# Liz490/multimodal_alzheimer

Hardware: AMD Instinct MI355X
Metric: volumes/sec fwd+bwd, 3D-ResNet-10 @128^3 bf16, 1/2/4/8 MI355X; % HBM roofline (higher is better)
Workload: dtype bf16; 1 GPU; BASELINE config 2: Anat_CNN ResNet-10 MRI-only, 1x128^3, batch 8/GPU, weighted CE, Adam, fwd+bwd+step; global_batch=8, parallelism=dp1, step_launch=hip graph replay

## Files before the change

include/mmad.h:

```cpp
#ifndef MMAD_H
#define MMAD_H

#include <stdint.h>

#ifdef __cplusplus
extern "C" {
#endif

enum { MMAD_OK = 0, MMAD_EBADSHAPE = 1001, MMAD_EBADDTYPE = 1002, MMAD_ENULL = 1003,
       MMAD_EUNSUPPORTED = 1004, MMAD_EHIP = 2000 };

enum { MMAD_F32 = 0, MMAD_BF16 = 1, MMAD_F64 = 2, MMAD_F16 = 3, MMAD_BITS = 4 };

typedef struct mmad_conv_desc {
  int32_t n;
  int32_t ci, di, hi, wi;
  int32_t co, do_, ho, wo;
  int32_t kd, kh, kw;
  int32_t sd, sh, sw;
  int32_t pd, ph, pw;
  int32_t dd, dh, dw;
} mmad_conv_desc;

int mmad_abi_version(void);
// ... 71 lines not shown
                      float* dw, float* dbias, void* workspace, void* stream);
int mmad_conv3d_wgrad_split(const mmad_conv_desc* d, int dtype, const void* x, const void* dy,
                            float* dw, float* dbias, void* workspace, void* stream,
                            void* reduce_stream);
int mmad_stem_raw_ok(const mmad_conv_desc* d, int in_dtype, int dtype);
int mmad_conv3d_fwd_raw(const mmad_conv_desc* d, int in_dtype, const void* x, int dtype,
                        const void* w_packed, const float* bias, void* y, float* stats,
                        void* stream);
typedef struct mmad_wgrad_job {
  const float* ws;
  float* dw;
  int32_t splits, nd, k, cs, taps, tper, kind, gx, gy, gz;
} mmad_wgrad_job;
int mmad_conv3d_wgrad_deferred(const mmad_conv_desc* d, int dtype, const void* x,
                               const void* dy, float* dw, void* workspace, mmad_wgrad_job* job,
                               void* stream);
int mmad_conv3d_wgrad_raw_deferred(const mmad_conv_desc* d, int in_dtype, const void* x,
                                   int dtype, const void* dy, float* dw, void* workspace,
                                   mmad_wgrad_job* job, void* stream);
int mmad_wgrad_reduce_batch(int njobs, const mmad_wgrad_job* jobs, void* stream);
int mmad_conv3d_wgrad_raw(const mmad_conv_desc* d, int in_dtype, const void* x, int dtype,
                          const void* dy, float* dw, float* dbias, void* workspace,
                          void* stream, void* reduce_stream);
int mmad_stem_dgrad_ok(const mmad_conv_desc* d, int dtype, int out_dtype);
int64_t mmad_stem_dgrad_ws_bytes(const mmad_conv_desc* d);
int mmad_conv3d_dgrad_raw(const mmad_conv_desc* d, int dtype, const void* dy, const float* w,
                          int out_dtype, void* dx, void* ws, void* stream);

int64_t mmad_bn_stats_parts(int64_t m, int c);
int mmad_bn_stats(int dtype, int64_t m, int c, const void* y, float* parts, void* stream);
int mmad_bn_parts_fold(int c, int nparts, const float* parts, int group, float* out,
                       void* stream);
int mmad_bn_finalize(int c, int64_t count, int nparts, const float* parts,
                     const float* gamma, const float* beta, float* running_mean,
                     float* running_var, float momentum, float eps, int training,
                     float* mean, float* invstd, float* scale, float* shift,
                     int64_t* num_batches_tracked, void* stream);
typedef struct mmad_bn_fin {
  int nparts;
  const float* parts;
  const float* gamma;
  const float* beta;
  float* running_mean;
  float* running_var;
  float momentum;
  float eps;
  int training;
  float* mean;
  float* invstd;
  float* scale;
  float* shift;
  int64_t* num_batches_tracked;
} mmad_bn_fin;
int mmad_bn_finalize2(int c, int64_t count, const mmad_bn_fin* a, const mmad_bn_fin* b,
                      void* stream);
int mmad_scale_shift_act(int dtype, int64_t m, int c, const void* y, const float* scale,
                         const float* shift, const void* res, const float* rscale,
                         const float* rshift, int relu, void* out, void* stream);
int64_t mmad_bn_bwd_parts(int64_t m, int c);
int mmad_bn_bwd_reduce(int dtype, int64_t m, int c, const void* g, const void* g2,
                       const void* relu_out, const void* y, const float* mean,
                       const float* invstd, float* parts, void* stream);
int mmad_bn_bwd_finalize(int c, int64_t count, int nparts, const float* parts,
                         const float* gamma, const float* invstd, int training,
                         float* dgamma, float* dbeta, float* coef, void* stream);
int mmad_bn_bwd_apply(int dtype, int64_t m, int c, const void* g, const void* g2,
                      const void* relu_out, const void* y, const float* mean,
                      const float* invstd, const float* coef, void* dy, void* gmask_out,
                      void* stream);
int mmad_bn_bwd_reduce2(int dtype, int64_t m, int c, const void* g, const void* g2,
                        int64_t g_rows, const void* relu_out, const void* y, const float* mean,
                        const float* invstd, const void* y2,
                        const float* mean2, const float* invstd2, float* parts, float* parts2,
                        void* stream);
int mmad_bn_bwd_finalize2(int c, int64_t count, int nparts, const float* parts,
                          const float* gamma, const float* invstd, int training, float* dgamma,
                          float* dbeta, float* coef, const float* parts2, const float* gamma2,
                          const float* invstd2, int training2, float* dgamma2, float* dbeta2,
                          float* coef2, void* stream);
int mmad_bn_bwd_apply2(int dtype, int64_t m, int c, const void* g, const void* g2,
                       int64_t g_rows, const void* relu_out, const void* y, const float* mean, const float* invstd, const float* coef,
                       void* dy, const void* y2, const float* mean2, const float* invstd2,
                       const float* coef2, void* dy2, void* stream);
int mmad_bn_relu_bwd_reduce(int dtype, int64_t m, int c, const void* g, const void* y,
                            const float* mean, const float* invstd, const float* scale,
                            const float* shift, float* parts, void* stream);
int mmad_bn_relu_bwd_apply(int dtype, int64_t m, int c, const void* g, const void* y,
                           const float* mean, const float* invstd, const float* scale,
                           const float* shift, const float* coef, void* dy, void* stream);
int mmad_relu_fwd(int dtype, int64_t n, const void* x, void* y, void* stream);
int mmad_relu_bwd(int dtype, int64_t n, const void* g, const void* out, void* dx, void* stream);
int mmad_add(int dtype, int64_t n, const void* a, const void* b, void* out, void* stream);

int mmad_colsum_ws(int dtype, int64_t m, int c, const void* y, float* parts, float* out,
                   void* stream);
int mmad_maxpool3d_fwd(int dtype, int n, int c, int di, int hi, int wi, int do_, int ho,
                       int wo, int k, int s, int p, const void* x, void* y,
                       uint8_t* argmax, void* stream);
int mmad_maxpool3d_bwd(int dtype, int n, int c, int di, int hi, int wi, int do_, int ho,
                       int wo, int k, int s, int p, const void* dy, const uint8_t* argmax,
                       void* dx, void* stream);
int mmad_bnpool_fwd(int dtype, int n, int c, int di, int hi, int wi, int do_, int ho, int wo,
                    int k, int s, int p, const void* y, const float* scale, const float* shift,
                    void* out, uint8_t* argmax, void* ymax, void* stream);
int mmad_bnpool_bwd_reduce(int dtype, int64_t m, int c, const void* g, const void* g2,
                           void* gsum, const uint8_t* argmax, const void* ymax,
                           const float* mean, const float* invstd, float* parts, void* stream);
int mmad_bnpool_bwd_apply(int dtype, int n, int c, int di, int hi, int wi, int do_, int ho,
                          int wo, int k, int s, int p, const void* g, const uint8_t* argmax,
                          const void* y, const float* mean, const float* invstd,
                          const float* coef, void* dy, void* stream);
int mmad_gap_fwd(int dtype, int n, int64_t s, int c, const void* x, float* y, void* stream);
int64_t mmad_gap_fwd_ws_elems(int n, int64_t s, int c);
int mmad_gap_fwd_ws(int dtype, int n, int64_t s, int c, const void* x, float* y, float* ws,
                    void* stream);
int mmad_gap_bwd(int dtype, int n, int64_t s, int c, const float* dy, void* dx, void* stream);
int mmad_gap_bwd_compact(int dtype, int n, int64_t s, int c, const float* dy, void* dx,
                         void* stream);
int mmad_gap_parts(int n, int64_t s, int c);
int mmad_gap_partial(int dtype, int n, int64_t s, int c, const void* x, float* ws,
                     void* stream);
int mmad_gap_linear_fwd(int b, int in, int out, int parts, int64_t s, const float* ws,
                        const float* w, const float* bias, int relu, float* xs, float* y,
                        void* stream);
int mmad_linear_gap_bwd(int b, int in, int out, int64_t s, const float* x, const float* w,
                        const float* dy, const float* ymask, int rows_dtype, void* rows,
                        float* dw, float* dbias, void* stream);

int mmad_linear_fwd(int b, int in, int out, const float* x, const float* w,
                    const float* bias, int relu, float* y, void* stream);
int mmad_linear_bwd(int b, int in, int out, const float* x, const float* w,
                    const float* dy, float* dx, float* dw, float* dbias, void* stream);
int mmad_linear_bwd_ex(int b, int in, int out, const float* x, const float* w,
                       const float* dy, const float* ymask, float* dx, float* dw, float* dbias,
                       void* stream);
int mmad_concat_cols(int b, int n_in, const float* const* srcs, const int* widths,
                     float* dst, void* stream);
int mmad_split_cols(int b, int n_out, const float* src, float* const* dsts,
                    const int* widths, void* stream);

int mmad_gather_channels(int in_dtype, int nsrc, const void* const* srcs,
                         int64_t batch_stride, int64_t vox_stride, int n, int64_t vox,
                         int cpad, int out_dtype, void* dst, void* stream);
int mmad_pad_rows(int rows, int cin, int cout, const float* src, float* dst, void* stream);
int mmad_take_channel(int in_dtype, int64_t rows, int cpad, int ch, const void* src,
                      int out_dtype, void* dst, void* stream);
int mmad_concat_channels(int dtype, int64_t rows, int ca, const void* a, int cb,
                         const void* b, void* dst, void* stream);
int mmad_split_channels(int dtype, int64_t rows, int ca, int cb, const void* src, void* a,
                        void* b, void* stream);
int mmad_max2_fwd(int dtype, int64_t n, const void* a, const void* b, void* y, uint8_t* sel,
                  void* stream);
int mmad_max2_bwd(int dtype, int64_t n, const void* g, const uint8_t* sel, void* ga, void* gb,
                  void* stream);

int mmad_cast(int in_dtype, int out_dtype, int64_t n, const void* x, void* y, void* stream);
int mmad_dropout_fwd(int dtype, int64_t n, float p, uint64_t seed, const void* x, void* y,
                     uint8_t* keep, void* stream);
int mmad_dropout_fwd_dev(int dtype, int64_t n, float p, const uint64_t* seed, const void* x,
                         void* y, uint8_t* keep, void* stream);
int mmad_dropout_bwd(int dtype, int64_t n, float p, const void* g, const uint8_t* keep,
                     void* dx, void* stream);

int mmad_loss_fwd(int b, int c, const double* logits, const int64_t* labels,
                  const double* weight, double gamma, int mode, double* loss,
                  double* dlogits, void* stream);
int mmad_loss_fwd_ex(int b, int c, int logits_dtype, const void* logits,
                     const int64_t* labels, const double* weight, double gamma, int mode,
                     double* logits64, double* loss, double* dlogits, void* stream);
int mmad_loss_bwd(int64_t n, const double* dlogits, const double* gloss, const double* gout,
                  int out_dtype, void* dx, void* stream);

int mmad_bootstrap_cls_metrics(int n, int c, const double* logits, const int64_t* labels,
                               int ndraw, const int64_t* idx, float* f1, float* mcc,
                               void* stream);
int mmad_mean_std(int n, const float* v, double* out, void* stream);

int64_t mmad_norm_ws_bytes(int nscan, int64_t vox);
int mmad_mri_minmax_norm(int nscan, int64_t vox, const double* x, const double* mask,
                         double q, double* out, void* ws, double* q_out, void* stream);
int mmad_mri_zscore_norm(int nscan, int64_t vox, const double* x, const double* mask,
                         double* out, void* ws, void* stream);
int mmad_affine_norm(int64_t n, const double* x, double mean, double stdv, double* out,
                     void* stream);

#define MMAD_AUG_MAX_MOD 4
typedef struct mmad_augment_cfg {
  double flip_p[3];
  double rot_max[3];
  double scale_lo, scale_hi;
  double trans_max[3];
  double gain_lo[MMAD_AUG_MAX_MOD], gain_hi[MMAD_AUG_MAX_MOD];
  double bias_lo[MMAD_AUG_MAX_MOD], bias_hi[MMAD_AUG_MAX_MOD];
  int32_t nmod, pad_;
} mmad_augment_cfg;
int mmad_augment_draw(int b, int d, int h, int w, const mmad_augment_cfg* cfg,
                      const uint64_t* seed, double* theta, double* intensity, void* stream);
enum { MMAD_PAD_ZEROS = 0, MMAD_PAD_BORDER = 1 };
int mmad_affine_resample3d(int b, int d, int h, int w, const double* x, const double* theta,
                           const double* gain_bias, int64_t gb_stride, int padding,
                           double* out, void* stream);

int64_t mmad_cache_stride_bytes(int kind, int64_t vox);
int64_t mmad_cache_ws_bytes(void);
// ... 16 lines not shown
```

multimodal_alzheimer_amd/_lib.py:

```python
import ctypes as C
import os

import torch

_PKG = os.path.dirname(os.path.abspath(__file__))
LIB_PATH = os.environ.get("MMAD_LIB_PATH") or os.path.join(_PKG, "libmmad_hip.so")

F32, BF16, F64 = 0, 1, 2
F16, BITS = 3, 4
EUNSUPPORTED = 1004
EHIP = 2000
_HIP_OOM = 2

_vp, _i32, _i64, _f32, _f64, _u64 = C.c_void_p, C.c_int, C.c_int64, C.c_float, C.c_double, C.c_uint64


class ConvDesc(C.Structure):
    _fields_ = [(n, C.c_int32) for n in (
        "n", "ci", "di", "hi", "wi", "co", "do_", "ho", "wo", "kd", "kh", "kw",
        "sd", "sh", "sw", "pd", "ph", "pw", "dd", "dh", "dw")]


class PackJob(C.Structure):
    _fields_ = ([("w", C.c_void_p), ("w_packed", C.c_void_p)] +
# ... 19 lines not shown
class BnFin(C.Structure):
    _fields_ = ([("nparts", C.c_int32)] +
                [(n, C.c_void_p) for n in ("parts", "gamma", "beta", "running_mean",
                                           "running_var")] +
                [("momentum", C.c_float), ("eps", C.c_float), ("training", C.c_int32)] +
                [(n, C.c_void_p) for n in ("mean", "invstd", "scale", "shift",
                                           "num_batches_tracked")])


class WgradJob(C.Structure):
    _fields_ = ([("ws", C.c_void_p), ("dw", C.c_void_p)] +
                [(n, C.c_int32) for n in ("splits", "nd", "k", "cs", "taps", "tper", "kind",
                                          "gx", "gy", "gz")])


AUG_MAX_MOD = 4
PAD_ZEROS, PAD_BORDER = 0, 1


class AugmentCfg(C.Structure):
    _fields_ = ([("flip_p", C.c_double * 3), ("rot_max", C.c_double * 3),
                 ("scale_lo", C.c_double), ("scale_hi", C.c_double),
                 ("trans_max", C.c_double * 3)] +
                [(n, C.c_double * AUG_MAX_MOD) for n in ("gain_lo", "gain_hi", "bias_lo",
                                                         "bias_hi")] +
                [("nmod", C.c_int32), ("pad_", C.c_int32)])


_P = C.POINTER(ConvDesc)
_PJ = C.POINTER(PackJob)
_PD = C.POINTER(PackDual)
_PA = C.POINTER(AdamJob)
_SIGS = {
    "mmad_abi_version": (_i32, []),
    "mmad_strerror": (C.c_char_p, [_i32]),
    "mmad_set_kernel_variant": (_i32, [C.c_char_p, _i32]),
    "mmad_conv_packed_elems": (_i64, [_P, _i32, _i32]),
    "mmad_conv_pack_weight": (_i32, [_P, _i32, _vp, _vp, _i32, _vp]),
    "mmad_conv_pack_job": (_i32, [_P, _i32, _i32, _vp, _vp, _i64, _PJ]),
    "mmad_pack_job_tiles": (_i64, [_PJ]),
    "mmad_conv_pack_batch": (_i32, [_i32, _i32, _vp, _i64, _vp]),
    "mmad_conv_pack_dual_job": (_i32, [_P, _i32, _vp, _vp, _vp, _i64, _PD]),
    "mmad_pack_dual_tiles": (_i64, [_PD]),
    "mmad_conv_pack_dual_batch": (_i32, [_i32, _i32, _vp, _i64, _vp]),
    "mmad_adam_job_tiles": (_i64, [_PA]),
    "mmad_adam_repack": (_i32, [_i32, _vp, _vp, _i64, _vp, _vp]),
    "mmad_conv_unfolded_elems": (_i64, [_P]),
    "mmad_conv_unfold_input": (_i32, [_P, _i32, _vp, _i32, _vp, _vp]),
    "mmad_conv3d_stats_rows": (_i64, [_P, _i32]),
    "mmad_conv3d_fwd": (_i32, [_P, _i32, _vp, _vp, _vp, _vp, _vp, _vp]),
    "mmad_conv3d_dgrad": (_i32, [_P, _i32, _vp, _vp, _vp, _vp]),
    "mmad_conv3d_dgrad_bnsum_rows": (_i64, [_P, _i32]),
    "mmad_conv3d_dgrad_bnsum": (_i32, [_P, _i32] + [_vp] * 10),
    "mmad_conv3d_wgrad_workspace": (_i64, [_P, _i32]),
    "mmad_conv3d_wgrad": (_i32, [_P, _i32, _vp, _vp, _vp, _vp, _vp, _vp]),
    "mmad_conv3d_wgrad_split": (_i32, [_P, _i32, _vp, _vp, _vp, _vp, _vp, _vp, _vp]),
    "mmad_conv3d_wgrad_deferred": (_i32, [_P, _i32, _vp, _vp, _vp, _vp,
                                          C.POINTER(WgradJob), _vp]),
    "mmad_conv3d_wgrad_raw_deferred": (_i32, [_P, _i32, _vp, _i32, _vp, _vp, _vp,
                                              C.POINTER(WgradJob), _vp]),
    "mmad_wgrad_reduce_batch": (_i32, [_i32, C.POINTER(WgradJob), _vp]),
    "mmad_stem_raw_ok": (_i32, [_P, _i32, _i32]),
    "mmad_conv3d_fwd_raw": (_i32, [_P, _i32, _vp, _i32, _vp, _vp, _vp, _vp, _vp]),
    "mmad_conv3d_wgrad_raw": (_i32, [_P, _i32, _vp, _i32, _vp, _vp, _vp, _vp, _vp, _vp]),
    "mmad_stem_dgrad_ok": (_i32, [_P, _i32, _i32]),
    "mmad_stem_dgrad_ws_bytes": (_i64, [_P]),
    "mmad_conv3d_dgrad_raw": (_i32, [_P, _i32, _vp, _vp, _i32, _vp, _vp, _vp]),
    "mmad_bn_stats_parts": (_i64, [_i64, _i32]),
    "mmad_bn_stats": (_i32, [_i32, _i64, _i32, _vp, _vp, _vp]),
    "mmad_bn_parts_fold": (_i32, [_i32, _i32, _vp, _i32, _vp, _vp]),
    "mmad_bn_finalize": (_i32, [_i32, _i64, _i32, _vp, _vp, _vp, _vp, _vp, _f32, _f32, _i32,
                                _vp, _vp, _vp, _vp, _vp, _vp]),
    "mmad_bn_finalize2": (_i32, [_i32, _i64, C.POINTER(BnFin), C.POINTER(BnFin), _vp]),
    "mmad_scale_shift_act": (_i32, [_i32, _i64, _i32, _vp, _vp, _vp, _vp, _vp, _vp, _i32, _vp,
                                    _vp]),
    "mmad_bn_bwd_parts": (_i64, [_i64, _i32]),
    "mmad_bn_bwd_reduce": (_i32, [_i32, _i64, _i32] + [_vp] * 8),
    "mmad_bn_bwd_finalize": (_i32, [_i32, _i64, _i32, _vp, _vp, _vp, _i32, _vp, _vp, _vp, _vp]),
    "mmad_bn_bwd_apply": (_i32, [_i32, _i64, _i32] + [_vp] * 10),
    "mmad_bn_bwd_reduce2": (_i32, [_i32, _i64, _i32, _vp, _vp, _i64] + [_vp] * 10),
    "mmad_bn_bwd_finalize2": (_i32, [_i32, _i64, _i32, _vp, _vp, _vp, _i32, _vp, _vp, _vp,
                                     _vp, _vp, _vp, _i32, _vp, _vp, _vp, _vp]),
    "mmad_bn_bwd_apply2": (_i32, [_i32, _i64, _i32, _vp, _vp, _i64] + [_vp] * 12),
    "mmad_relu_fwd": (_i32, [_i32, _i64, _vp, _vp, _vp]),
    "mmad_relu_bwd": (_i32, [_i32, _i64, _vp, _vp, _vp, _vp]),
    "mmad_colsum_ws": (_i32, [_i32, _i64, _i32, _vp, _vp, _vp, _vp]),
    "mmad_add": (_i32, [_i32, _i64, _vp, _vp, _vp, _vp]),
    "mmad_maxpool3d_fwd": (_i32, [_i32] * 12 + [_vp, _vp, _vp, _vp]),
    "mmad_maxpool3d_bwd": (_i32, [_i32] * 12 + [_vp, _vp, _vp, _vp]),
    "mmad_bnpool_fwd": (_i32, [_i32] * 12 + [_vp] * 7),
    "mmad_bnpool_bwd_reduce": (_i32, [_i32, _i64, _i32] + [_vp] * 9),
    "mmad_bnpool_bwd_apply": (_i32, [_i32] * 12 + [_vp] * 8),
    "mmad_gap_fwd": (_i32, [_i32, _i32, _i64, _i32, _vp, _vp, _vp]),
    "mmad_gap_fwd_ws_elems": (_i64, [_i32, _i64, _i32]),
    "mmad_conv3d_fwd_ex": (_i32, [_P, _i32, _vp, _vp, _vp, _vp, _i32, _vp, _vp, _vp]),
    "mmad_conv_pack_weight_scaled": (_i32, [_P, _i32, _vp, _vp, _vp, _i32, _vp]),
    "mmad_bn_fold": (_i32, [_i32, _vp, _vp, _vp, _vp, _f32, _vp, _vp, _vp, _vp]),
    "mmad_norm_ws_bytes": (_i64, [_i32, _i64]),
    "mmad_mri_minmax_norm": (_i32, [_i32, _i64, _vp, _vp, _f64, _vp, _vp, _vp, _vp]),
    "mmad_mri_zscore_norm": (_i32, [_i32, _i64, _vp, _vp, _vp, _vp, _vp]),
    "mmad_affine_norm": (_i32, [_i64, _vp, _f64, _f64, _vp, _vp]),
    "mmad_gap_fwd_ws": (_i32, [_i32, _i32, _i64, _i32, _vp, _vp, _vp, _vp]),
    "mmad_gap_bwd": (_i32, [_i32, _i32, _i64, _i32, _vp, _vp, _vp]),
    "mmad_gap_bwd_compact": (_i32, [_i32, _i32, _i64, _i32, _vp, _vp, _vp]),
    "mmad_gap_parts": (_i32, [_i32, _i64, _i32]),
    "mmad_gap_partial": (_i32, [_i32, _i32, _i64, _i32, _vp, _vp, _vp]),
    "mmad_gap_linear_fwd": (_i32, [_i32, _i32, _i32, _i32, _i64, _vp, _vp, _vp, _i32, _vp,
                                   _vp, _vp]),
    "mmad_linear_gap_bwd": (_i32, [_i32, _i32, _i32, _i64, _vp, _vp, _vp, _vp, _i32, _vp, _vp,
                                   _vp, _vp]),
    "mmad_linear_fwd": (_i32, [_i32, _i32, _i32, _vp, _vp, _vp, _i32, _vp, _vp]),
    "mmad_linear_bwd": (_i32, [_i32, _i32, _i32, _vp, _vp, _vp, _vp, _vp, _vp, _vp]),
    "mmad_linear_bwd_ex": (_i32, [_i32, _i32, _i32] + [_vp] * 8),
    "mmad_concat_cols": (_i32, [_i32, _i32, _vp, _vp, _vp, _vp]),
    "mmad_split_cols": (_i32, [_i32, _i32, _vp, _vp, _vp, _vp]),
    "mmad_cast": (_i32, [_i32, _i32, _i64, _vp, _vp, _vp]),
    "mmad_dropout_fwd": (_i32, [_i32, _i64, _f32, _u64, _vp, _vp, _vp, _vp]),
    "mmad_dropout_fwd_dev": (_i32, [_i32, _i64, _f32, _vp, _vp, _vp, _vp, _vp]),
    "mmad_dropout_bwd": (_i32, [_i32, _i64, _f32, _vp, _vp, _vp, _vp]),
    "mmad_loss_fwd": (_i32, [_i32, _i32, _vp, _vp, _vp, _f64, _i32, _vp, _vp, _vp]),
    "mmad_loss_fwd_ex": (_i32, [_i32, _i32, _i32, _vp, _vp, _vp, _f64, _i32, _vp, _vp, _vp,
                                _vp]),
    "mmad_loss_bwd": (_i32, [_i64, _vp, _vp, _vp, _i32, _vp, _vp]),
    "mmad_gather_channels": (_i32, [_i32, _i32, _vp, _i64, _i64, _i32, _i64, _i32, _i32, _vp,
                                    _vp]),
    "mmad_pad_rows": (_i32, [_i32, _i32, _i32, _vp, _vp, _vp]),
    "mmad_take_channel": (_i32, [_i32, _i64, _i32, _i32, _vp, _i32, _vp, _vp]),
    "mmad_concat_channels": (_i32, [_i32, _i64, _i32, _vp, _i32, _vp, _vp, _vp]),
    "mmad_split_channels": (_i32, [_i32, _i64, _i32, _i32, _vp, _vp, _vp, _vp]),
    "mmad_max2_fwd": (_i32, [_i32, _i64, _vp, _vp, _vp, _vp, _vp]),
    "mmad_max2_bwd": (_i32, [_i32, _i64, _vp, _vp, _vp, _vp, _vp]),
    "mmad_bootstrap_cls_metrics": (_i32, [_i32, _i32, _vp, _vp, _i32, _vp, _vp, _vp, _vp]),
    "mmad_mean_std": (_i32, [_i32, _vp, _vp, _vp]),
    "mmad_bn_relu_bwd_reduce": (_i32, [_i32, _i64, _i32] + [_vp] * 8),
    "mmad_bn_relu_bwd_apply": (_i32, [_i32, _i64, _i32] + [_vp] * 9),
    "mmad_augment_draw": (_i32, [_i32, _i32, _i32, _i32, C.POINTER(AugmentCfg), _vp, _vp, _vp,
                                 _vp]),
    "mmad_affine_resample3d": (_i32, [_i32, _i32, _i32, _i32, _vp, _vp, _vp, _i64, _i32, _vp,
                                      _vp]),
    "mmad_cache_stride_bytes": (_i64, [_i32, _i64]),
    "mmad_cache_ws_bytes": (_i64, []),
    "mmad_cache_store": (_i32, [_i32, _i32, _i64, _vp, _vp, _i64, _i64, _vp, _vp, _vp]),
    "mmad_cache_pack_mask": (_i32, [_i32, _i64, _vp, _vp, _i64, _i64, _vp, _vp, _vp]),
    "mmad_cache_fetch": (_i32, [_i32, _i32, _i64] + [_i32] * 6 + [_vp, _vp, _vp, _i64, _vp, _vp,
                                                                 _vp]),
    "mmad_cache_fetch_rows": (_i32, [_i32, _i64, _i32, _vp, _vp, _vp, _vp, _i64, _vp, _vp, _vp,
                                     _vp]),
}
EXPORTS = tuple(_SIGS)

_lib = None


class MMADError(RuntimeError):
    pass


def load():
    global _lib
    if _lib is None:
        if not os.path.exists(LIB_PATH):
            raise MMADError(f"{LIB_PATH} is missing: build it with "
                            "`python -m multimodal_alzheimer_amd._build` (hipcc, gfx950)")
        lib = C.CDLL(LIB_PATH)
        for name, (res, args) in _SIGS.items():
            fn = getattr(lib, name)
            fn.restype, fn.argtypes = res, args
        if lib.mmad_abi_version() != 1:
            raise MMADError("libmmad_hip.so ABI version mismatch")
        _lib = lib
    return _lib


def check(rc, what=""):
    if rc == 0:
        return
    msg = load().mmad_strerror(rc).decode()
    if rc == EHIP + _HIP_OOM:
        raise torch.OutOfMemoryError(f"{what}: {msg}")
    raise MMADError(f"{what} failed ({rc}): {msg}")


def call(name, *args):
    check(getattr(load(), name)(*args), name)


_cur_dev = torch._C._cuda_getDevice
_raw_stream = torch._C._cuda_getCurrentRawStream

# ... 29 lines not shown
```

multimodal_alzheimer_amd/csrc/bn.hip:

```cpp
#include "common.h"

constexpr int COLSUM_ROWS = 4;

namespace {

struct PartPlan {
  int64_t rpp;
  int nparts;
};
PartPlan part_plan(int64_t M) {
  int n = (int)std::min<int64_t>(1024, std::max<int64_t>(1, cdiv(M, 64)));
  const int64_t rpp = cdiv(M, n);
  return {rpp, (int)cdiv(M, rpp)};
}

#ifndef BN_FOLD_PROBE
#define BN_FOLD_PROBE 0
#endif
#if BN_FOLD_PROBE
__device__ int g_fold_cnt[4096];
__device__ float g_fold_sink[4096];
#endif

template <typename T, int MODE, int V, bool DUAL = false, bool G2 = false, bool GB = false>
__global__ __launch_bounds__(256) void colsum_kernel(int64_t M, int C, int64_t rpp,
                                                     const T* __restrict__ y,
                                                     const T* __restrict__ g,
                                                     const T* __restrict__ relu_out,
                                                     const float* __restrict__ mean,
                                                     const float* __restrict__ invstd,
                                                     float* __restrict__ parts,
                                                     const uint8_t* __restrict__ act,
                                                     const float* __restrict__ msc,
                                                     const float* __restrict__ msh,
                                                     const T* __restrict__ y2 = nullptr,
                                                     const float* __restrict__ mean2 = nullptr,
                                                     const float* __restrict__ invstd2 = nullptr,
                                                     float* __restrict__ parts2 = nullptr,
                                                     const T* __restrict__ g2 = nullptr,
                                                     T* __restrict__ gsum = nullptr,
                                                     uint32_t gS = 0) {
  static_assert(!DUAL || MODE == 1, "dual partial sums: BN backward with a relu_out mask");
  static_assert(!GB || (DUAL && V == Chunk<T>::N), "broadcast g: the pair kernel, 16-byte rows");
  __shared__ float red[DUAL ? 3 : 2][2048];
  const int tid = threadIdx.x;
  const int CC = C / (int)gridDim.y;
  const int cb = (int)blockIdx.y * CC;
  const int lpr = CC / V;
  const int rpar = 256 / lpr;
  const int cl = tid % lpr, rl = tid / lpr;
  const int64_t r0 = (int64_t)blockIdx.x * rpp;
  const int64_t r1 = min(M, r0 + rpp);
  float s[V], q[V], q2[V];
#pragma unroll
  for (int e = 0; e < V; ++e) { s[e] = 0.f; q[e] = 0.f; q2[e] = 0.f; }
  if (rl < rpar) {
    float mu[V], is[V], sc[V], sh[V], mu2[V], is2[V];
    if (MODE == 1 || MODE == 3 || MODE == 4) {
#pragma unroll
      for (int e = 0; e < V; ++e) { mu[e] = mean[cb + cl * V + e]; is[e] = invstd[cb + cl * V + e]; }
    }
    if constexpr (DUAL) {
#pragma unroll
      for (int e = 0; e < V; ++e) {
        mu2[e] = mean2[cb + cl * V + e];
        is2[e] = invstd2[cb + cl * V + e];
      }
    }
    if (MODE == 4) {
#pragma unroll
      for (int e = 0; e < V; ++e) { sc[e] = msc[cb + cl * V + e]; sh[e] = msh[cb + cl * V + e]; }
    }
    auto accum = [&](int64_t i, float* yv, float* gv, const float* ov, const float* y2v) {
      if (MODE == 1 || MODE == 3 || MODE == 4) {
        if (MODE == 4) {
#pragma unroll
          for (int e = 0; e < V; ++e) gv[e] = bn_affine(yv[e], sc[e], sh[e]) > 0.f ? gv[e] : 0.f;
        } else if (MODE == 3) {
#pragma unroll
          for (int e = 0; e < V; ++e) gv[e] = (act[i + e] & 0x80) ? gv[e] : 0.f;
        } else if (relu_out != nullptr) {
#pragma unroll
          for (int e = 0; e < V; ++e) gv[e] = ov[e] > 0.f ? gv[e] : 0.f;
        }
#pragma unroll
        for (int e = 0; e < V; ++e) {
          s[e] += gv[e];
          q[e] += gv[e] * ((yv[e] - mu[e]) * is[e]);
        }
        if constexpr (DUAL) {
#pragma unroll
          for (int e = 0; e < V; ++e) q2[e] += gv[e] * ((y2v[e] - mu2[e]) * is2[e]);
        }
      } else {
#pragma unroll
        for (int e = 0; e < V; ++e) {
          s[e] += yv[e];
          if (MODE == 0) q[e] += yv[e] * yv[e];
        }
      }
    };
    constexpr bool NEED_G = MODE == 1 || MODE == 3 || MODE == 4;
    int64_t r = r0 + rl;
    if constexpr (V == Chunk<T>::N) {
      constexpr int U = COLSUM_ROWS;
      for (; r + (U - 1) * rpar < r1; r += U * rpar) {
        u32x4 yr[U], gr[U], orr[U], y2r[U], g2r[U];
#pragma unroll
        for (int u = 0; u < U; ++u) {
          const int64_t i = (r + u * rpar) * C + cb + cl * V;
          yr[u] = *reinterpret_cast<const u32x4*>(y + i);
          if constexpr (GB)
            gr[u] = *reinterpret_cast<const u32x4*>(
                g + (int64_t)((uint32_t)(r + u * rpar) / gS) * C + cb + cl * V);
          else if (NEED_G)
            gr[u] = *reinterpret_cast<const u32x4*>(g + i);
          if (NEED_G && G2) g2r[u] = *reinterpret_cast<const u32x4*>(g2 + i);
          if (MODE == 1 && relu_out != nullptr)
            orr[u] = *reinterpret_cast<const u32x4*>(relu_out + i);
          if constexpr (DUAL) y2r[u] = *reinterpret_cast<const u32x4*>(y2 + i);
        }
#pragma unroll
        for (int u = 0; u < U; ++u) {
          const int64_t i = (r + u * rpar) * C + cb + cl * V;
          float yv[V], gv[V], ov[V], y2v[V];
          Chunk<T>::load(reinterpret_cast<const T*>(&yr[u]), yv);
          if (NEED_G) Chunk<T>::load(reinterpret_cast<const T*>(&gr[u]), gv);
          if constexpr (NEED_G && G2) {
            float hv[V];
            Chunk<T>::load(reinterpret_cast<const T*>(&g2r[u]), hv);
#pragma unroll
            for (int e = 0; e < V; ++e) gv[e] = as_stored<T>(gv[e] + hv[e]);
            if constexpr (MODE == 3) Chunk<T>::store(gsum + i, gv);
          }
          if (MODE == 1 && relu_out != nullptr)
            Chunk<T>::load(reinterpret_cast<const T*>(&orr[u]), ov);
          if constexpr (DUAL) Chunk<T>::load(reinterpret_cast<const T*>(&y2r[u]), y2v);
          accum(i, yv, gv, ov, y2v);
        }
      }
    }
    for (; r < r1; r += rpar) {
      const int64_t i = r * C + cb + cl * V;
      float yv[V], gv[V], ov[V], y2v[V];
      if constexpr (V == Chunk<T>::N) Chunk<T>::load(y + i, yv);
      else for (int e = 0; e < V; ++e) yv[e] = Elt<T>::ld(y, i + e);
      if (NEED_G) {
        if constexpr (GB) Chunk<T>::load(g + (int64_t)((uint32_t)r / gS) * C + cb + cl * V, gv);
        else if constexpr (V == Chunk<T>::N) Chunk<T>::load(g + i, gv);
        else for (int e = 0; e < V; ++e) gv[e] = Elt<T>::ld(g, i + e);
        if constexpr (G2) {
          float hv[V];
          if constexpr (V == Chunk<T>::N) Chunk<T>::load(g2 + i, hv);
          else for (int e = 0; e < V; ++e) hv[e] = Elt<T>::ld(g2, i + e);
#pragma unroll
          for (int e = 0; e < V; ++e) gv[e] = as_stored<T>(gv[e] + hv[e]);
          if constexpr (MODE == 3) {
            if constexpr (V == Chunk<T>::N) Chunk<T>::store(gsum + i, gv);
            else for (int e = 0; e < V; ++e) Elt<T>::st(gsum, i + e, gv[e]);
          }
        }
        if (MODE == 1 && relu_out != nullptr) {
          if constexpr (V == Chunk<T>::N) Chunk<T>::load(relu_out + i, ov);
          else for (int e = 0; e < V; ++e) ov[e] = Elt<T>::ld(relu_out, i + e);
        }
      }
      if constexpr (DUAL) {
        if constexpr (V == Chunk<T>::N) Chunk<T>::load(y2 + i, y2v);
        else for (int e = 0; e < V; ++e) y2v[e] = Elt<T>::ld(y2, i + e);
      }
      accum(i, yv, gv, ov, y2v);
    }
#pragma unroll
    for (int e = 0; e < V; ++e) {
      red[0][rl * CC + cl * V + e] = s[e];
      red[1][rl * CC + cl * V + e] = q[e];
      if constexpr (DUAL) red[DUAL ? 2 : 0][rl * CC + cl * V + e] = q2[e];
    }
  }
  __syncthreads();
  for (int c = tid; c < CC; c += 256) {
    float ss = 0.f, qq = 0.f, q2q = 0.f;
    for (int k = 0; k < rpar; ++k) {
      ss += red[0][k * CC + c];
      qq += red[1][k * CC + c];
      if constexpr (DUAL) q2q += red[DUAL ? 2 : 0][k * CC + c];
    }
    parts[((int64_t)blockIdx.x * 2) * C + cb + c] = ss;
    parts[((int64_t)blockIdx.x * 2 + 1) * C + cb + c] = qq;
    if constexpr (DUAL) {
      parts2[((int64_t)blockIdx.x * 2) * C + cb + c] = ss;
      parts2[((int64_t)blockIdx.x * 2 + 1) * C + cb + c] = q2q;
    }
  }
#if BN_FOLD_PROBE
  __shared__ int last;
  const int ngx = ((int)gridDim.x + 31) >> 5;
  const int grp = (int)blockIdx.y * ngx + ((int)blockIdx.x >> 5);
  const int gsize = min(32, (int)gridDim.x - (((int)blockIdx.x >> 5) << 5));
  __threadfence();
  __syncthreads();
  if (tid == 0) last = atomicAdd(&g_fold_cnt[grp & 4095], 1) == gsize - 1;
  __syncthreads();
  if (last) {
    __threadfence();
    for (int c = tid; c < CC; c += 256) {
      float ss = 0.f, qq = 0.f;
      const int p0 = ((int)blockIdx.x >> 5) << 5;
      for (int k = 0; k < gsize; ++k) {
        ss += parts[((int64_t)(p0 + k) * 2) * C + cb + c];
        qq += parts[((int64_t)(p0 + k) * 2 + 1) * C + cb + c];
      }
      g_fold_sink[(grp * 64 + c) & 4095] = ss + qq;
    }
    if (tid == 0) g_fold_cnt[grp & 4095] = 0;
  }
#endif
}

__global__ void parts_fold_kernel(int C, int nparts, int group, const float* __restrict__ in,
                                  float* __restrict__ out) {
  const int o = blockIdx.x;
  for (int c = threadIdx.x; c < 2 * C; c += blockDim.x) {
    float s = 0.f;
    const int p1 = min(nparts, (o + 1) * group);
#pragma unroll 8
    for (int p = o * group; p < p1; ++p) s += in[(int64_t)p * 2 * C + c];
    out[(int64_t)o * 2 * C + c] = s;
  }
}

template <typename T, int MODE>
int launch_colsum(int64_t M, int C, const void* y, const void* g, const void* ro,
                  const float* mean, const float* invstd, float* parts, hipStream_t st,
                  const uint8_t* act = nullptr, const float* msc = nullptr,
                  const float* msh = nullptr, const void* g2 = nullptr,
                  void* gsum = nullptr) {
  const PartPlan pp = part_plan(M);
  constexpr int VEC = Chunk<T>::N;
  dim3 grid((unsigned)pp.nparts);
  int slabs = 1;
  while (C % (slabs * 2 * VEC) == 0 && C / (slabs * VEC) > 256) slabs *= 2;
#define COLSUM(VV, G)                                                                       \
  hipLaunchKernelGGL((colsum_kernel<T, MODE, VV, false, G>), grid, dim3(256), 0, st, M, C, \
                     pp.rpp, (const T*)y, (const T*)g, (const T*)ro, mean, invstd, parts, act, \
// ... 137 lines not shown
  if (conv_bias) sh += conv_bias[c] * sc;
  scale[c] = sc;
  bias[c] = sh;
}

__device__ __forceinline__ void bwd_finalize(int C, int64_t count, int nparts,
                                             const float* parts, const float* gamma,
                                             const float* invstd, int training, float* dgamma,
                                             float* dbeta, float* coef, double* sm) {
  const int c = blockIdx.x * FC + (threadIdx.x % FC);
  const bool own = threadIdx.x < FC && c < C;
  float gm = 1.f, is = 0.f;
  if (own) {
    if (gamma) gm = gamma[c];
    is = invstd[c];
  }
  double S, Q;
  sum_parts(c, C, nparts, parts, sm, S, Q);
  if (!own) return;
  if (dbeta) dbeta[c] = (float)S;
  if (dgamma) dgamma[c] = (float)Q;
  const double k0 = (double)gm * is;
  coef[c] = (float)k0;
  coef[C + c] = training ? (float)(k0 * S / (double)count) : 0.f;
  coef[2 * C + c] = training ? (float)(k0 * Q / (double)count) : 0.f;
}

__global__ __launch_bounds__(1024) void bn_bwd_finalize_kernel(
    int C, int64_t count, int nparts, const float* __restrict__ parts,
    const float* __restrict__ gamma, const float* __restrict__ invstd, int training,
    float* dgamma, float* dbeta, float* coef) {
  __shared__ double sm[2048];
  bwd_finalize(C, count, nparts, parts, gamma, invstd, training, dgamma, dbeta, coef, sm);
}

struct BwdFin {
  const float* parts;
  const float* gamma;
  const float* invstd;
  int training;
  float* dgamma;
  float* dbeta;
  float* coef;
};

__global__ __launch_bounds__(1024) void bn_bwd_finalize2_kernel(int C, int64_t count,
                                                                int nparts, BwdFin a, BwdFin b) {
  __shared__ double sm[2048];
  const BwdFin& f = blockIdx.y ? b : a;
  bwd_finalize(C, count, nparts, f.parts, f.gamma, f.invstd, f.training, f.dgamma, f.dbeta,
               f.coef, sm);
}

__global__ void sum_only_finalize_kernel(int C, int nparts, const float* __restrict__ parts,
                                         float* out) {
  __shared__ double sm[2048];
  const int c = blockIdx.x * FC + (threadIdx.x % FC);
  double S, Q;
  sum_parts(c, C, nparts, parts, sm, S, Q);
  if (threadIdx.x >= FC || c >= C) return;
  out[c] = (float)S;
}

template <typename T, int RES>
__global__ void scale_shift_act_kernel(int64_t M, int C, const T* __restrict__ y,
                                       const float* __restrict__ scale,
                                       const float* __restrict__ shift,
                                       const T* __restrict__ res,
                                       const float* __restrict__ rscale,
                                       const float* __restrict__ rshift, int relu,
                                       T* __restrict__ out) {
  constexpr int N = Chunk<T>::N;
  const int64_t nchunks = M * C / N;
  for (int64_t q = blockIdx.x * (int64_t)blockDim.x + threadIdx.x; q < nchunks;
       q += (int64_t)gridDim.x * blockDim.x) {
    const int64_t i0 = q * N;
    const int c0 = (int)(i0 % C);
    float v[N], r[N];
    Chunk<T>::load(y + i0, v);
    if (RES) Chunk<T>::load(res + i0, r);
#pragma unroll
    for (int e = 0; e < N; ++e) {
      const int c = c0 + e;
      float o = bn_affine(v[e], scale[c], shift[c]);
      if (RES == 1) o += r[e];
      if (RES == 2) o += r[e] * rscale[c] + rshift[c];
      v[e] = relu ? fmaxf(o, 0.f) : o;
    }
    Chunk<T>::store(out + i0, v);
  }
}

template <int N>
__device__ __forceinline__ void ld_params(const float* __restrict__ p, float* v) {
#pragma unroll
  for (int h = 0; h < N / 4; ++h) {
    const f32x4 c = *reinterpret_cast<const f32x4*>(p + 4 * h);
    v[4 * h] = c[0]; v[4 * h + 1] = c[1]; v[4 * h + 2] = c[2]; v[4 * h + 3] = c[3];
  }
}

template <typename T, int RES>
__global__ __launch_bounds__(256) void scale_shift_act_fc_kernel(
    int64_t nchunks, int cpr, const T* __restrict__ y, const float* __restrict__ scale,
    const float* __restrict__ shift, const T* __restrict__ res, const float* __restrict__ rscale,
    const float* __restrict__ rshift, int relu, T* __restrict__ out) {
  constexpr int N = Chunk<T>::N;
  const int64_t t0 = (int64_t)blockIdx.x * 256 + threadIdx.x;
  const int64_t stride = (int64_t)gridDim.x * 256;
  const int c0 = (int)(t0 & (cpr - 1)) * N;
  float sc[N], sh[N], rs[N], rh[N];
  ld_params<N>(scale + c0, sc);
  ld_params<N>(shift + c0, sh);
  if (RES == 2) {
    ld_params<N>(rscale + c0, rs);
    ld_params<N>(rshift + c0, rh);
  }
  auto apply = [&](float* v, const float* r) {
#pragma unroll
    for (int e = 0; e < N; ++e) {
      float o = bn_affine(v[e], sc[e], sh[e]);
      if (RES == 1) o += r[e];
      if (RES == 2) o += r[e] * rs[e] + rh[e];
      v[e] = relu ? fmaxf(o, 0.f) : o;
    }
  };
  int64_t q = t0;
  for (; q + stride < nchunks; q += 2 * stride) {
    float v0[N], v1[N], r0[N], r1[N];
    Chunk<T>::load(y + q * N, v0);
    Chunk<T>::load(y + (q + stride) * N, v1);
    if (RES) {
      Chunk<T>::load(res + q * N, r0);
      Chunk<T>::load(res + (q + stride) * N, r1);
    }
    apply(v0, r0);
    apply(v1, r1);
    Chunk<T>::store(out + q * N, v0);
    Chunk<T>::store(out + (q + stride) * N, v1);
  }
  if (q < nchunks) {
    float v0[N], r0[N];
    Chunk<T>::load(y + q * N, v0);
    if (RES) Chunk<T>::load(res + q * N, r0);
    apply(v0, r0);
    Chunk<T>::store(out + q * N, v0);
  }
}

template <typename T>
__global__ void scale_shift_act_scalar_kernel(int64_t M, int C, const T* __restrict__ y,
                                              const float* __restrict__ scale,
                                              const float* __restrict__ shift,
                                              const T* __restrict__ res,
                                              const float* __restrict__ rscale,
                                              const float* __restrict__ rshift, int relu,
                                              T* __restrict__ out) {
  const int64_t n = M * C;
  for (int64_t i = blockIdx.x * (int64_t)blockDim.x + threadIdx.x; i < n;
       i += (int64_t)gridDim.x * blockDim.x) {
    const int c = (int)(i % C);
    float o = bn_affine(Elt<T>::ld(y, i), scale[c], shift[c]);
    if (res) o += rscale ? Elt<T>::ld(res, i) * rscale[c] + rshift[c] : Elt<T>::ld(res, i);
    Elt<T>::st(out, i, relu ? fmaxf(o, 0.f) : o);
  }
}

struct BwdApply2 {
  const void* y2;
  const float* mean2;
  const float* invstd2;
  const float* coef2;
  void* dy2;
};

template <typename T, bool MASKY = false, bool DUAL = false, bool G2 = false, bool GB = false>
__global__ __launch_bounds__(256) void bn_bwd_apply_fc_kernel(
    int64_t nv, int cpr, int C, const T* __restrict__ g, const T* __restrict__ relu_out,
    const T* __restrict__ y, const float* __restrict__ mean, const float* __restrict__ invstd,
    const float* __restrict__ coef, T* __restrict__ dy, T* __restrict__ gmask,
    const float* __restrict__ msc = nullptr, const float* __restrict__ msh = nullptr,
    BwdApply2 d2 = {}, const T* __restrict__ g2 = nullptr, uint32_t gS = 0) {
  constexpr int V = Chunk<T>::N;
  const int cpr_shift = __builtin_ctz(cpr);
  auto g_at = [&](int64_t qq) -> const T* {
    if constexpr (GB)
      return g + (int64_t)((uint32_t)(qq >> cpr_shift) / gS) * C + (qq & (cpr - 1)) * V;
    else
      return g + qq * V;
  };
  const int64_t t0 = (int64_t)blockIdx.x * 256 + threadIdx.x;
  const int64_t stride = (int64_t)gridDim.x * 256;
  const int c0 = (int)(t0 & (cpr - 1)) * V;
  float mu[V], is[V], k0[V], k1[V], k2[V];
  ld_params<V>(mean + c0, mu);
  ld_params<V>(invstd + c0, is);
  ld_params<V>(coef + c0, k0);
  ld_params<V>(coef + C + c0, k1);
  ld_params<V>(coef + 2 * C + c0, k2);
  float sc[V], sh[V];
  if constexpr (MASKY) {
    ld_params<V>(msc + c0, sc);
    ld_params<V>(msh + c0, sh);
  }
  const T* __restrict__ y2 = static_cast<const T*>(d2.y2);
  T* __restrict__ dy2 = static_cast<T*>(d2.dy2);
  float mu2[V], is2[V], j0[V], j1[V], j2[V];
  if constexpr (DUAL) {
    ld_params<V>(d2.mean2 + c0, mu2);
    ld_params<V>(d2.invstd2 + c0, is2);
    ld_params<V>(d2.coef2 + c0, j0);
    ld_params<V>(d2.coef2 + C + c0, j1);
    ld_params<V>(d2.coef2 + 2 * C + c0, j2);
  }
  auto one = [&](int64_t q, const float* gv0, const float* yv, const float* ov,
                 const float* y2v) {
    float gv[V], dv[V], dv2[V];
#pragma unroll
    for (int e = 0; e < V; ++e) {
      if constexpr (MASKY) gv[e] = bn_affine(yv[e], sc[e], sh[e]) > 0.f ? gv0[e] : 0.f;
      else gv[e] = (relu_out && !(ov[e] > 0.f)) ? 0.f : gv0[e];
      const float xh = (yv[e] - mu[e]) * is[e];
      dv[e] = k0[e] * gv[e] - k1[e] - xh * k2[e];
      if constexpr (DUAL) {
        const float xh2 = (y2v[e] - mu2[e]) * is2[e];
        dv2[e] = j0[e] * gv[e] - j1[e] - xh2 * j2[e];
      }
    }
    Chunk<T>::store(dy + q * V, dv);
    if constexpr (DUAL) Chunk<T>::store(dy2 + q * V, dv2);
    if (gmask) Chunk<T>::store(gmask + q * V, gv);
  };
  auto add_g2 = [&](int64_t qq, float* gv) {
    float hv[V];
    Chunk<T>::load(g2 + qq * V, hv);
#pragma unroll
    for (int e = 0; e < V; ++e) gv[e] = as_stored<T>(gv[e] + hv[e]);
  };
  int64_t q = t0;
  for (; q + stride < nv; q += 2 * stride) {
    float g0[V], g1[V], y0[V], y1[V], o0[V], o1[V], z0[V], z1[V];
    Chunk<T>::load(g_at(q), g0);
    Chunk<T>::load(g_at(q + stride), g1);
    if constexpr (G2) {
      add_g2(q, g0);
      add_g2(q + stride, g1);
    }
    Chunk<T>::load(y + q * V, y0);
    Chunk<T>::load(y + (q + stride) * V, y1);
    if (relu_out) {
      Chunk<T>::load(relu_out + q * V, o0);
      Chunk<T>::load(relu_out + (q + stride) * V, o1);
    }
    if constexpr (DUAL) {
      Chunk<T>::load(y2 + q * V, z0);
      Chunk<T>::load(y2 + (q + stride) * V, z1);
    }
    one(q, g0, y0, o0, z0);
    one(q + stride, g1, y1, o1, z1);
  }
  if (q < nv) {
    float g0[V], y0[V], o0[V], z0[V];
    Chunk<T>::load(g_at(q), g0);
    if constexpr (G2) add_g2(q, g0);
    Chunk<T>::load(y + q * V, y0);
    if (relu_out) Chunk<T>::load(relu_out + q * V, o0);
    if constexpr (DUAL) Chunk<T>::load(y2 + q * V, z0);
    one(q, g0, y0, o0, z0);
  }
}

template <typename T, int V>
__global__ void bn_bwd_apply_kernel(int64_t M, int C, const T* __restrict__ g,
                                    const T* __restrict__ relu_out, const T* __restrict__ y,
                                    const float* __restrict__ mean,
                                    const float* __restrict__ invstd,
                                    const float* __restrict__ coef, T* __restrict__ dy,
                                    T* __restrict__ gmask) {
  const int64_t nv = M * C / V;
  for (int64_t q = blockIdx.x * (int64_t)blockDim.x + threadIdx.x; q < nv;
       q += (int64_t)gridDim.x * blockDim.x) {
    const int64_t i = q * V;
    const int c0 = (int)(i % C);
    float gv[V], yv[V], ov[V], dv[V];
    if constexpr (V == Chunk<T>::N) {
      Chunk<T>::load(g + i, gv);
      Chunk<T>::load(y + i, yv);
      if (relu_out) Chunk<T>::load(relu_out + i, ov);
    } else {
      for (int e = 0; e < V; ++e) {
        gv[e] = Elt<T>::ld(g, i + e);
        yv[e] = Elt<T>::ld(y, i + e);
        if (relu_out) ov[e] = Elt<T>::ld(relu_out, i + e);
      }
    }
#pragma unroll
    for (int e = 0; e < V; ++e) {
      const int c = c0 + e;
      if (relu_out && !(ov[e] > 0.f)) gv[e] = 0.f;
      const float xh = (yv[e] - mean[c]) * invstd[c];
      dv[e] = coef[c] * gv[e] - coef[C + c] - xh * coef[2 * C + c];
    }
    if constexpr (V == Chunk<T>::N) {
      Chunk<T>::store(dy + i, dv);
      if (gmask) Chunk<T>::store(gmask + i, gv);
    } else {
      for (int e = 0; e < V; ++e) {
        Elt<T>::st(dy, i + e, dv[e]);
        if (gmask) Elt<T>::st(gmask, i + e, gv[e]);
      }
    }
  }
}

template <typename T>
__global__ void relu_bwd_kernel(int64_t n, const T* __restrict__ g, const T* __restrict__ out,
                                T* __restrict__ dx) {
  for (int64_t i = blockIdx.x * (int64_t)blockDim.x + threadIdx.x; i < n;
       i += (int64_t)gridDim.x * blockDim.x)
    Elt<T>::st(dx, i, Elt<T>::ld(out, i) > 0.f ? Elt<T>::ld(g, i) : 0.f);
}

template <typename T>
__global__ void relu_fwd_kernel(int64_t n, const T* __restrict__ x, T* __restrict__ y) {
  for (int64_t i = blockIdx.x * (int64_t)blockDim.x + threadIdx.x; i < n;
       i += (int64_t)gridDim.x * blockDim.x) {
    const float v = Elt<T>::ld(x, i);
    Elt<T>::st(y, i, v > 0.f ? v : (v != v ? v : 0.f));
  }
}

template <typename T>
__global__ void add_kernel(int64_t n, const T* __restrict__ a, const T* __restrict__ b,
                           T* __restrict__ o) {
  for (int64_t i = blockIdx.x * (int64_t)blockDim.x + threadIdx.x; i < n;
       i += (int64_t)gridDim.x * blockDim.x)
    Elt<T>::st(o, i, Elt<T>::ld(a, i) + Elt<T>::ld(b, i));
}

unsigned ew_grid(int64_t n) {
  return (unsigned)std::max<int64_t>(1, std::min<int64_t>(cdiv(n, 256), 256 * 16));
}

bool dt_ok(int dtype) { return dtype == MMAD_F32 || dtype == MMAD_BF16; }

}

extern "C" {

int64_t mmad_bn_stats_parts(int64_t m, int c) {
  (void)c;
  return m > 0 ? part_plan(m).nparts : -1;
}
int64_t mmad_bn_bwd_parts(int64_t m, int c) { return mmad_bn_stats_parts(m, c); }

int mmad_bn_stats(int dtype, int64_t m, int c, const void* y, float* parts, void* stream) {
  if (!dt_ok(dtype)) return MMAD_EBADDTYPE;
  if (m <= 0 || c <= 0) return MMAD_EBADSHAPE;
  if (!y || !parts) return MMAD_ENULL;
  if (dtype == MMAD_BF16)
    return launch_colsum<u16, 0>(m, c, y, nullptr, nullptr, nullptr, nullptr, parts,
                                 as_stream(stream));
  return launch_colsum<float, 0>(m, c, y, nullptr, nullptr, nullptr, nullptr, parts,
                                 as_stream(stream));
}

int mmad_bn_parts_fold(int c, int nparts, const float* parts, int group, float* out,
                       void* stream) {
  if (c <= 0 || nparts <= 0 || group <= 0) return MMAD_EBADSHAPE;
  if (!parts || !out) return MMAD_ENULL;
  hipLaunchKernelGGL(parts_fold_kernel, dim3((unsigned)cdiv(nparts, group)), dim3(256), 0,
                     as_stream(stream), c, nparts, group, parts, out);
  return launch_status();
}

int mmad_colsum_ws(int dtype, int64_t m, int c, const void* y, float* parts, float* out,
                   void* stream) {
  if (!dt_ok(dtype)) return MMAD_EBADDTYPE;
  if (m <= 0 || c <= 0) return MMAD_EBADSHAPE;
  if (!y || !parts || !out) return MMAD_ENULL;
  int rc = dtype == MMAD_BF16
               ? launch_colsum<u16, 2>(m, c, y, nullptr, nullptr, nullptr, nullptr, parts,
                                       as_stream(stream))
               : launch_colsum<float, 2>(m, c, y, nullptr, nullptr, nullptr, nullptr, parts,
                                         as_stream(stream));
  if (rc) return rc;
  hipLaunchKernelGGL(sum_only_finalize_kernel, dim3((unsigned)cdiv(c, FC)), dim3(1024), 0,
                     as_stream(stream), c, part_plan(m).nparts, parts, out);
  return launch_status();
}

int mmad_bn_finalize2(int c, int64_t count, const mmad_bn_fin* a, const mmad_bn_fin* b,
                      void* stream) {
  if (c <= 0 || count <= 0) return MMAD_EBADSHAPE;
  if (!a || !b) return MMAD_ENULL;
  for (const mmad_bn_fin* f : {a, b}) {
    if (f->training && (!f->parts || f->nparts <= 0)) return MMAD_ENULL;
    if (!f->training && (!f->running_mean || !f->running_var)) return MMAD_ENULL;
  }
  hipLaunchKernelGGL(bn_finalize2_kernel, dim3((unsigned)cdiv(c, FC), 2), dim3(1024), 0,
                     as_stream(stream), c, count, *a, *b);
  return launch_status();
}

int mmad_bn_finalize(int c, int64_t count, int nparts, const float* parts, const float* gamma,
                     const float* beta, float* running_mean, float* running_var,
                     float momentum, float eps, int training, float* mean, float* invstd,
                     float* scale, float* shift, int64_t* num_batches_tracked, void* stream) {
  if (c <= 0 || count <= 0) return MMAD_EBADSHAPE;
  if (training && (!parts || nparts <= 0)) return MMAD_ENULL;
  if (!training && (!running_mean || !running_var)) return MMAD_ENULL;
  hipLaunchKernelGGL(bn_finalize_kernel, dim3((unsigned)cdiv(c, FC)), dim3(1024), 0,
                     as_stream(stream), c, count, nparts, parts, gamma, beta, running_mean,
                     running_var, momentum, eps, training, mean, invstd, scale, shift,
                     num_batches_tracked);
  return launch_status();
}

int mmad_scale_shift_act(int dtype, int64_t m, int c, const void* y, const float* scale,
                         const float* shift, const void* res, const float* rscale,
                         const float* rshift, int relu, void* out, void* stream) {
  if (!dt_ok(dtype)) return MMAD_EBADDTYPE;
  if (m <= 0 || c <= 0) return MMAD_EBADSHAPE;
  if (!y || !scale || !shift || !out) return MMAD_ENULL;
  if ((rscale == nullptr) != (rshift == nullptr)) return MMAD_ENULL;
  hipStream_t st = as_stream(stream);
  const int epc = dtype == MMAD_BF16 ? 8 : 4;
  const int rk = res == nullptr ? 0 : (rscale == nullptr ? 1 : 2);
// ... 74 lines not shown
  else
    hipLaunchKernelGGL((bn_bwd_apply_fc_kernel<float, true>), dim3(ew_grid(nv)), dim3(256), 0,
                       st, nv, c / vv, c, (const float*)g, (const float*)nullptr,
                       (const float*)y, mean, invstd, coef, (float*)dy, (float*)nullptr, scale,
                       shift);
  return launch_status();
}

int mmad_bnpool_bwd_reduce(int dtype, int64_t m, int c, const void* g, const void* g2,
                           void* gsum, const uint8_t* argmax, const void* ymax,
                           const float* mean, const float* invstd, float* parts,
                           void* stream) {
  if (!dt_ok(dtype)) return MMAD_EBADDTYPE;
  if (m <= 0 || c <= 0) return MMAD_EBADSHAPE;
  if (!g || !argmax || !ymax || !mean || !invstd || !parts) return MMAD_ENULL;
  if (g2 && !gsum) return MMAD_ENULL;
  if (dtype == MMAD_BF16)
    return launch_colsum<u16, 3>(m, c, ymax, g, nullptr, mean, invstd, parts, as_stream(stream),
                                 argmax, nullptr, nullptr, g2, gsum);
  return launch_colsum<float, 3>(m, c, ymax, g, nullptr, mean, invstd, parts, as_stream(stream),
                                 argmax, nullptr, nullptr, g2, gsum);
}

int mmad_bn_fold(int c, const float* gamma, const float* beta, const float* running_mean,
                 const float* running_var, float eps, const float* conv_bias, float* scale,
                 float* bias, void* stream) {
  if (c <= 0) return MMAD_EBADSHAPE;
  if (!running_mean || !running_var || !scale || !bias) return MMAD_ENULL;
  hipLaunchKernelGGL(bn_fold_kernel, dim3((unsigned)cdiv(c, 256)), dim3(256), 0,
                     as_stream(stream), c, gamma, beta, running_mean, running_var, eps, conv_bias,
                     scale, bias);
  return launch_status();
}

int mmad_bn_bwd_finalize(int c, int64_t count, int nparts, const float* parts,
                         const float* gamma, const float* invstd, int training, float* dgamma,
                         float* dbeta, float* coef, void* stream) {
  if (c <= 0 || count <= 0 || nparts <= 0) return MMAD_EBADSHAPE;
  if (!parts || !invstd || !coef) return MMAD_ENULL;
  hipLaunchKernelGGL(bn_bwd_finalize_kernel, dim3((unsigned)cdiv(c, FC)), dim3(1024), 0,
                     as_stream(stream), c, count, nparts, parts, gamma, invstd, training,
                     dgamma, dbeta, coef);
  return launch_status();
}

int mmad_bn_bwd_apply(int dtype, int64_t m, int c, const void* g, const void* g2,
                      const void* relu_out, const void* y, const float* mean,
                      const float* invstd, const float* coef, void* dy, void* gmask,
                      void* stream) {
  if (!dt_ok(dtype)) return MMAD_EBADDTYPE;
  if (m <= 0 || c <= 0) return MMAD_EBADSHAPE;
  if (!g || !y || !mean || !invstd || !coef || !dy) return MMAD_ENULL;
  hipStream_t st = as_stream(stream);
#define APPLY(T, V)                                                                          \
  hipLaunchKernelGGL((bn_bwd_apply_kernel<T, V>), dim3(ew_grid(m * c / V)), dim3(256), 0, st, \
                     m, c, (const T*)g, (const T*)relu_out, (const T*)y, mean, invstd, coef,  \
                     (T*)dy, (T*)gmask)
  const int vv = dtype == MMAD_BF16 ? 8 : 4;
  if (c % vv == 0 && is_pow2(c / vv) && c / vv <= 256) {
    const int64_t nv = m * c / vv;
#define APPLYFC(T, G)                                                                         \
  hipLaunchKernelGGL((bn_bwd_apply_fc_kernel<T, false, false, G>), dim3(ew_grid(nv)), dim3(256), \
                     0, st, nv, c / vv, c, (const T*)g, (const T*)relu_out, (const T*)y, mean,  \
                     invstd, coef, (T*)dy, (T*)gmask, nullptr, nullptr, BwdApply2{},           \
                     (const T*)g2)
    if (dtype == MMAD_BF16) {
      if (g2 != nullptr) APPLYFC(u16, true); else APPLYFC(u16, false);
    } else {
      if (g2 != nullptr) APPLYFC(float, true); else APPLYFC(float, false);
    }
#undef APPLYFC
    return launch_status();
  }
  if (g2 != nullptr) return MMAD_EUNSUPPORTED;
  if (dtype == MMAD_BF16) {
    if (c % 8 == 0) APPLY(u16, 8); else APPLY(u16, 1);
  } else {
    if (c % 4 == 0) APPLY(float, 4); else APPLY(float, 1);
  }
#undef APPLY
  return launch_status();
}

int mmad_bn_bwd_reduce2(int dtype, int64_t m, int c, const void* g, const void* g2,
                        int64_t g_rows, const void* relu_out, const void* y, const float* mean,
                        const float* invstd, const void* y2,
                        const float* mean2, const float* invstd2, float* parts, float* parts2,
                        void* stream) {
  if (!dt_ok(dtype)) return MMAD_EBADDTYPE;
  if (m <= 0 || c <= 0) return MMAD_EBADSHAPE;
  if (!g || !relu_out || !y || !mean || !invstd || !y2 || !mean2 || !invstd2 || !parts ||
      !parts2)
    return MMAD_ENULL;
  if (g_rows < 0 || (g_rows > 0 && (m % g_rows || m >= (int64_t(1) << 31))))
    return MMAD_EBADSHAPE;
  const PartPlan pp = part_plan(m);
  hipStream_t st = as_stream(stream);
  auto go = [&](auto tag) -> int {
    using T = decltype(tag);
    constexpr int VEC = Chunk<T>::N;
    int slabs = 1;
    while (c % (slabs * 2 * VEC) == 0 && c / (slabs * VEC) > 256) slabs *= 2;
    if (!(c % (slabs * VEC) == 0 && c / (slabs * VEC) <= 256)) return MMAD_EUNSUPPORTED;
    auto k = g_rows > 0 ? (g2 != nullptr ? colsum_kernel<T, 1, VEC, true, true, true>
                                          : colsum_kernel<T, 1, VEC, true, false, true>)
                        : (g2 != nullptr ? colsum_kernel<T, 1, VEC, true, true>
                                          : colsum_kernel<T, 1, VEC, true, false>);
    hipLaunchKernelGGL(k, dim3((unsigned)pp.nparts, slabs), dim3(256), 0, st, m, c, pp.rpp,
                       (const T*)y, (const T*)g, (const T*)relu_out, mean, invstd, parts,
                       nullptr, nullptr, nullptr, (const T*)y2, mean2, invstd2, parts2,
                       (const T*)g2, (T*)nullptr, (uint32_t)g_rows);
    return launch_status();
  };
  return dtype == MMAD_BF16 ? go(u16{}) : go(float{});
}

int mmad_bn_bwd_finalize2(int c, int64_t count, int nparts, const float* parts,
                          const float* gamma, const float* invstd, int training, float* dgamma,
                          float* dbeta, float* coef, const float* parts2, const float* gamma2,
                          const float* invstd2, int training2, float* dgamma2, float* dbeta2,
                          float* coef2, void* stream) {
  if (c <= 0 || count <= 0 || nparts <= 0) return MMAD_EBADSHAPE;
  if (!parts || !invstd || !coef || !parts2 || !invstd2 || !coef2) return MMAD_ENULL;
  const BwdFin a{parts, gamma, invstd, training, dgamma, dbeta, coef};
  const BwdFin b{parts2, gamma2, invstd2, training2, dgamma2, dbeta2, coef2};
  hipLaunchKernelGGL(bn_bwd_finalize2_kernel, dim3((unsigned)cdiv(c, FC), 2), dim3(1024), 0,
                     as_stream(stream), c, count, nparts, a, b);
  return launch_status();
}

int mmad_bn_bwd_apply2(int dtype, int64_t m, int c, const void* g, const void* g2,
                       int64_t g_rows, const void* relu_out, const void* y, const float* mean, const float* invstd, const float* coef,
                       void* dy, const void* y2, const float* mean2, const float* invstd2,
                       const float* coef2, void* dy2, void* stream) {
  if (!dt_ok(dtype)) return MMAD_EBADDTYPE;
  if (m <= 0 || c <= 0) return MMAD_EBADSHAPE;
  if (!g || !relu_out || !y || !mean || !invstd || !coef || !dy || !y2 || !mean2 || !invstd2 ||
      !coef2 || !dy2)
    return MMAD_ENULL;
  const int vv = dtype == MMAD_BF16 ? 8 : 4;
  if (!(c % vv == 0 && is_pow2(c / vv) && c / vv <= 256)) return MMAD_EUNSUPPORTED;
  const int64_t nv = m * c / vv;
  const BwdApply2 d2{y2, mean2, invstd2, coef2, dy2};
  hipStream_t st = as_stream(stream);
  if (g_rows < 0 || (g_rows > 0 && (m % g_rows || m >= (int64_t(1) << 31))))
    return MMAD_EBADSHAPE;
#define APPLY2(T, G, B)                                                                      \
  hipLaunchKernelGGL((bn_bwd_apply_fc_kernel<T, false, true, G, B>), dim3(ew_grid(nv)),       \
                     dim3(256), 0, st, nv, c / vv, c, (const T*)g, (const T*)relu_out,        \
                     (const T*)y, mean, invstd, coef, (T*)dy, (T*)nullptr, nullptr, nullptr,  \
                     d2, (const T*)g2, (uint32_t)g_rows)
#define APPLY2G(T, B)                                                                        \
  do {                                                                                       \
    if (g2 != nullptr) APPLY2(T, true, B); else APPLY2(T, false, B);                         \
  } while (0)
  if (dtype == MMAD_BF16) {
    if (g_rows > 0) APPLY2G(u16, true); else APPLY2G(u16, false);
  } else {
    if (g_rows > 0) APPLY2G(float, true); else APPLY2G(float, false);
  }
#undef APPLY2G
#undef APPLY2
  return launch_status();
}

int mmad_relu_bwd(int dtype, int64_t n, const void* g, const void* out, void* dx, void* stream) {
  if (!dt_ok(dtype)) return MMAD_EBADDTYPE;
  if (n <= 0) return MMAD_EBADSHAPE;
  if (!g || !out || !dx) return MMAD_ENULL;
  if (dtype == MMAD_BF16)
    hipLaunchKernelGGL(relu_bwd_kernel<u16>, dim3(ew_grid(n)), dim3(256), 0, as_stream(stream),
                       n, (const u16*)g, (const u16*)out, (u16*)dx);
  else
    hipLaunchKernelGGL(relu_bwd_kernel<float>, dim3(ew_grid(n)), dim3(256), 0,
                       as_stream(stream), n, (const float*)g, (const float*)out, (float*)dx);
  return launch_status();
}

int mmad_relu_fwd(int dtype, int64_t n, const void* x, void* y, void* stream) {
  if (!dt_ok(dtype)) return MMAD_EBADDTYPE;
  if (n <= 0) return MMAD_EBADSHAPE;
  if (!x || !y) return MMAD_ENULL;
  if (dtype == MMAD_BF16)
    hipLaunchKernelGGL(relu_fwd_kernel<u16>, dim3(ew_grid(n)), dim3(256), 0, as_stream(stream),
                       n, (const u16*)x, (u16*)y);
  else
    hipLaunchKernelGGL(relu_fwd_kernel<float>, dim3(ew_grid(n)), dim3(256), 0,
                       as_stream(stream), n, (const float*)x, (float*)y);
  return launch_status();
}

int mmad_add(int dtype, int64_t n, const void* a, const void* b, void* out, void* stream) {
  if (!dt_ok(dtype)) return MMAD_EBADDTYPE;
  if (n <= 0) return MMAD_EBADSHAPE;
  if (!a || !b || !out) return MMAD_ENULL;
  if (dtype == MMAD_BF16)
    hipLaunchKernelGGL(add_kernel<u16>, dim3(ew_grid(n)), dim3(256), 0, as_stream(stream), n,
                       (const u16*)a, (const u16*)b, (u16*)out);
  else
    hipLaunchKernelGGL(add_kernel<float>, dim3(ew_grid(n)), dim3(256), 0, as_stream(stream), n,
                       (const float*)a, (const float*)b, (float*)out);
  return launch_status();
}

}
```

multimodal_alzheimer_amd/csrc/common.h:

```cpp
#pragma once
#include <hip/hip_runtime.h>
#include <stdint.h>

#include "../../include/mmad.h"

typedef float f32x4 __attribute__((ext_vector_type(4)));
typedef __bf16 bf16x8 __attribute__((ext_vector_type(8)));
typedef __bf16 bf16x4 __attribute__((ext_vector_type(4)));
typedef unsigned short u16;
typedef unsigned short u16x8 __attribute__((ext_vector_type(8)));
typedef unsigned short u16x4 __attribute__((ext_vector_type(4)));
typedef uint32_t u32x4 __attribute__((ext_vector_type(4)));

#define LDS_AS __attribute__((address_space(3)))

template <int N>
__device__ __forceinline__ void wait_vm_lgkm0() {
  static_assert(N >= 0 && N <= 63, "vmcnt immediate (6 bits)");
  asm volatile("s_waitcnt vmcnt(%0) lgkmcnt(0)" ::"i"(N) : "memory");
}

__device__ __forceinline__ void raw_barrier() {
  __builtin_amdgcn_s_barrier();
  asm volatile("" ::: "memory");
// ... 16 lines not shown
      "buffer_load_dwordx4 %1, %2, 0 offen lds\n\ts_mov_b32 m0, %0"
      : "=&s"(keep)
      : "v"(voff), "s"(rsrc), "s"(lds_addr)
      : "memory");
}
__device__ __forceinline__ uint32_t lds_addr_of(const void* p) {
  return __builtin_amdgcn_readfirstlane((uint32_t)(uintptr_t)(const LDS_AS void*)p);
}

__device__ __forceinline__ float bf2f(u16 v) { return __uint_as_float(((uint32_t)v) << 16); }
typedef float f32x2 __attribute__((ext_vector_type(2)));
typedef __bf16 bf16x2 __attribute__((ext_vector_type(2)));
__device__ __forceinline__ uint32_t pack_bf16x2(float a, float b) {
  return __builtin_bit_cast(uint32_t, __builtin_convertvector((f32x2){a, b}, bf16x2));
}
__device__ __forceinline__ u16 f2bf(float f) { return (u16)(pack_bf16x2(f, 0.f) & 0xffffu); }

template <typename T> struct Elt;
template <> struct Elt<float> {
  static __device__ __forceinline__ float ld(const float* p, int64_t i) { return p[i]; }
  static __device__ __forceinline__ void st(float* p, int64_t i, float v) { p[i] = v; }
  static constexpr int VEC = 4;
};
template <> struct Elt<u16> {
  static __device__ __forceinline__ float ld(const u16* p, int64_t i) { return bf2f(p[i]); }
  static __device__ __forceinline__ void st(u16* p, int64_t i, float v) { p[i] = f2bf(v); }
  static constexpr int VEC = 8;
};

template <typename T> struct Chunk;
template <> struct Chunk<float> {
  static constexpr int N = 4;
  static __device__ __forceinline__ void load(const float* p, float* v) {
    f32x4 c = *reinterpret_cast<const f32x4*>(p);
    v[0] = c[0]; v[1] = c[1]; v[2] = c[2]; v[3] = c[3];
  }
  static __device__ __forceinline__ void store(float* p, const float* v) {
    f32x4 c; c[0] = v[0]; c[1] = v[1]; c[2] = v[2]; c[3] = v[3];
    *reinterpret_cast<f32x4*>(p) = c;
  }
};
template <> struct Chunk<u16> {
  static constexpr int N = 8;
  static __device__ __forceinline__ void load(const u16* p, float* v) {
    u16x8 c = *reinterpret_cast<const u16x8*>(p);
#pragma unroll
    for (int i = 0; i < 8; ++i) v[i] = bf2f(c[i]);
  }
  static __device__ __forceinline__ void store(u16* p, const float* v) {
    u32x4 c;
#pragma unroll
    for (int i = 0; i < 4; ++i) c[i] = pack_bf16x2(v[2 * i], v[2 * i + 1]);
    *reinterpret_cast<u32x4*>(p) = c;
  }
};

__device__ __forceinline__ u32x4 epi_res_relu(u32x4 v, const u16* res, int relu) {
  float f[8];
  Chunk<u16>::load(reinterpret_cast<const u16*>(&v), f);
  if (res != nullptr) {
    float r[8];
    Chunk<u16>::load(res, r);
#pragma unroll
    for (int e = 0; e < 8; ++e) f[e] += r[e];
  }
  if (relu) {
#pragma unroll
    for (int e = 0; e < 8; ++e) f[e] = fmaxf(f[e], 0.f);
  }
  u32x4 o;
  Chunk<u16>::store(reinterpret_cast<u16*>(&o), f);
  return o;
}

__device__ __forceinline__ float bn_affine(float y, float scale, float shift) {
  return __builtin_fmaf(y, scale, shift);
}
template <typename T>
__device__ __forceinline__ float as_stored(float v) {
  if constexpr (sizeof(T) == 2) return bf2f(f2bf(v));
  else return v;
}

__device__ __forceinline__ float wave_sum(float v) {
#pragma unroll
  for (int o = 32; o > 0; o >>= 1) v += __shfl_xor(v, o, 64);
  return v;
}
__device__ __forceinline__ double wave_sum_d(double v) {
#pragma unroll
  for (int o = 32; o > 0; o >>= 1) v += __shfl_xor(v, o, 64);
  return v;
}

__device__ __forceinline__ uint64_t mix64(uint64_t z) {
  z += 0x9E3779B97F4A7C15ull;
  z = (z ^ (z >> 30)) * 0xBF58476D1CE4E5B9ull;
  z = (z ^ (z >> 27)) * 0x94D049BB133111EBull;
  return z ^ (z >> 31);
}

static inline int hip_status(hipError_t e) { return e == hipSuccess ? MMAD_OK : MMAD_EHIP + (int)e; }
static inline int launch_status() { return hip_status(hipGetLastError()); }
static inline hipStream_t as_stream(void* s) { return reinterpret_cast<hipStream_t>(s); }
static inline int64_t cdiv(int64_t a, int64_t b) { return (a + b - 1) / b; }

__global__ void zero_fill_kernel(uint32_t* __restrict__ p, int64_t words);
int zero_fill(void* p, int64_t bytes, hipStream_t st);
static inline bool is_pow2(int64_t v) { return v > 0 && (v & (v - 1)) == 0; }
static inline int ilog2(int64_t v) { int r = 0; while ((int64_t(1) << r) < v) ++r; return r; }
```

multimodal_alzheimer_amd/csrc/conv.hip:

```cpp
#include <cstring>

#include "common.h"
#include "reduce.h"
#include "patchconv.h"
#include "pointwise.h"
#include "stem.h"

namespace {

constexpr int MAXTAPS = 344;
constexpr int TAPB = ((3 * MAXTAPS * 4 + 15) / 16) * 16;
constexpr int RB = 128;

struct Geom {
  int M, Nd, Cs, K, Kpad, cs_shift, taps, nb;
  int Ds, Hs, Ws, Dd, Hd, Wd;
  int KD, KH, KW;
  int sd, sh, sw, pd, ph, pw, dd, dh, dw;
  const void* res;
  int relu;
};

enum { FWD = 0, DGRAD = 1 };

// ... 1346 lines not shown
  return launch_wgrad_k<T, BMW, 32, 2>(g, sp, x, dy, ws, st);
}

unsigned grid_for(int64_t total, int block = 256) {
  return (unsigned)std::max<int64_t>(1, std::min<int64_t>(cdiv(total, block), 65536));
}

enum Leaf { STEM, LATTICE5, LATTICE_ZP, LATTICE, LATTICE8, PATCHZ, PATCH, S2, PW, IGEMM, NONE };
enum Epi { EPI_NONE, EPI_RES, EPI_BNSUM };
bool leaf_has(Leaf l, Epi e) {
  if (e == EPI_RES) return l != STEM && l != PW;
  if (e == EPI_BNSUM) return l == LATTICE_ZP || l == LATTICE8 || l == PATCH;
  return true;
}
struct Route { Leaf leaf; int64_t tiles; };

Route resolve(const mmad_conv_desc* d, const Geom& g, int dtype, Epi epi, bool launch = true) {
  const Route none{NONE, -1};
  auto pick = [&](Leaf l, int64_t tiles) { return leaf_has(l, epi) ? Route{l, tiles} : none; };
  const bool u = d != nullptr && unfolded(d);
  if (u && epi != EPI_NONE) return none;
  if (u && mmad_stem::fwd_ok(d, dtype) && stem_kernel_on())
    return pick(STEM, mmad_stem::fwd_stats_rows(d));
  if (launch && !geom_ok(g, dtype)) return none;
  if (!u && dtype == MMAD_BF16) {
    const mmad_patch::Geo q = patch_geo(g);
    if (g.sd == 1 && g.sh == 1 && g.sw == 1) {
      if (mmad_lattice5::ok(q)) return pick(LATTICE5, mmad_lattice5::tiles(q));
      const bool zp = mmad_lattice_zp::ok(q);
      const int64_t lt = zp ? mmad_lattice_zp::tiles(q) : mmad_lattice::tiles(q);
      if (mmad_lattice::ok(q, lt)) return pick(zp ? LATTICE_ZP : LATTICE, lt);
      if (mmad_lattice8::ok(q)) return pick(LATTICE8, mmad_lattice8::tiles(q));
      if (mmad_patch::ok(q))
        return mmad_patchz::ok(q) ? pick(PATCHZ, mmad_patchz::tiles(q))
                                  : pick(PATCH, mmad_patch::tiles(q));
    }
    if (mmad_s2::ok(q, g.sd, g.sh, g.sw)) return pick(S2, mmad_s2::tiles(q));
  }
  if (d != nullptr && leaf_has(PW, epi) && mmad_pw::fwd_ok(d, dtype))
    return pick(PW, mmad_pw::fwd_tiles(d));
  return pick(IGEMM, cdiv(g.M, fwd_tile_rows(g, dtype)));
}

int launch_route(const Route& r, const mmad_conv_desc* d, const Geom& g, int dtype,
                 const mmad_patch::Geo& q, const void* x, const void* wp, const float* bias,
                 void* y, float* stats, void* stream) {
  switch (r.leaf) {
    case STEM: return mmad_stem::fwd(d, x, wp, bias, y, stats, stream);
    case LATTICE5: return mmad_lattice5::fwd(q, x, wp, bias, y, stats, stream);
    case LATTICE_ZP: return mmad_lattice_zp::fwd(q, x, wp, bias, y, stats, stream);
    case LATTICE: return mmad_lattice::fwd(q, x, wp, bias, y, stats, stream);
    case LATTICE8: return mmad_lattice8::fwd(q, x, wp, bias, y, stats, stream);
    case PATCHZ: return mmad_patchz::fwd(q, x, wp, bias, y, stats, stream);
    case PATCH: return mmad_patch::fwd(q, x, wp, bias, y, stats, stream);
    case S2: return mmad_s2::fwd(q, g.sd, g.sh, g.sw, x, wp, bias, y, stats, stream);
    case PW: return mmad_pw::fwd(d, x, wp, bias, y, stats, stream);
    case IGEMM: return run_igemm<FWD>(g, dtype, g.M, 1, x, wp, bias, y, stats, as_stream(stream));
    case NONE: break;
  }
  return MMAD_EUNSUPPORTED;
}

Route dgrad_fwd_route(const mmad_conv_desc* d, int dtype, Epi epi, Geom* gf) {
  if (!desc_ok(d) || (dtype != MMAD_F32 && dtype != MMAD_BF16) || unfolded(d) ||
      mmad_pw::ok(d, dtype) || !dgrad_as_fwd(d))
    return Route{NONE, -1};
  *gf = dgrad_fwd_geom(d, dtype);
  return resolve(nullptr, *gf, dtype, epi);
}

}

extern "C" {

int mmad_set_kernel_variant(const char* name, int value) {
  if (name == nullptr) return -1;
  if (std::strcmp(name, "lattice_zp") == 0) return mmad_lattice_zp::set_mode(value);
  if (std::strcmp(name, "lattice") == 0) return mmad_lattice::set_mode(value);
  if (std::strcmp(name, "lattice8") == 0) return mmad_lattice8::set_mode(value);
  if (std::strcmp(name, "lattice5") == 0) return mmad_lattice5::set_mode(value);
  if (std::strcmp(name, "pool_run") == 0) return mmad_pool::set_run_mode(value);
  if (std::strcmp(name, "patchz") == 0) return mmad_patchz::set_mode(value);
  if (std::strcmp(name, "pw_wg3_dedup") == 0) return mmad_pw::set_wg3_dedup(value);
  return -1;
}

int64_t mmad_conv_packed_elems(const mmad_conv_desc* d, int dtype, int for_dgrad) {
  if (!desc_ok(d)) return -1;
  const Geom g = for_dgrad ? dgrad_geom(d, dtype) : fwd_geom(d, dtype);
  return (int64_t)g.Nd * g.Kpad;
}

int mmad_conv_pack_weight_scaled(const mmad_conv_desc* d, int dtype, const float* w,
                                 const float* scale, void* wp, int for_dgrad, void* stream);

int mmad_conv_pack_weight(const mmad_conv_desc* d, int dtype, const float* w, void* wp,
                          int for_dgrad, void* stream) {
  return mmad_conv_pack_weight_scaled(d, dtype, w, nullptr, wp, for_dgrad, stream);
}

int mmad_conv_pack_weight_scaled(const mmad_conv_desc* d, int dtype, const float* w,
                                 const float* scale, void* wp, int for_dgrad, void* stream) {
  if (!desc_ok(d)) return MMAD_EBADSHAPE;
  if (dtype != MMAD_F32 && dtype != MMAD_BF16) return MMAD_EBADDTYPE;
  if (!w || !wp) return MMAD_ENULL;
  if (for_dgrad && unfolded(d)) return MMAD_EUNSUPPORTED;
  const Geom g = for_dgrad ? dgrad_geom(d, dtype) : fwd_geom(d, dtype);
  if (!geom_ok(g, dtype)) return MMAD_EUNSUPPORTED;
  const int mode = for_dgrad ? 1 : (unfolded(d) ? 2 : 0);
  const int flip = for_dgrad && dgrad_as_fwd(d);
  const int64_t total = (int64_t)g.Nd * g.Kpad;
  if (scale != nullptr && (mode != 0 || g.Kpad != g.K)) return MMAD_EUNSUPPORTED;
  if (mode != 2 && g.Kpad == g.K) {
    const int R = mode == 0 ? d->ci : d->co;
    const int Cc = mode == 0 ? g.taps : d->ci * g.taps;
    const int B = mode == 0 ? d->co : 1;
    const int64_t ob = mode == 0 ? g.Kpad : 0, oj1 = mode == 0 ? 0 : g.Kpad;
    const int jd = g.taps, oj2 = mode == 0 ? d->ci : d->co;
    dim3 grid((unsigned)cdiv(Cc, 64), (unsigned)cdiv(R, 64), (unsigned)B);
    if (dtype == MMAD_BF16)
      hipLaunchKernelGGL(pack_transpose_kernel<u16>, grid, dim3(256), 0, as_stream(stream), w,
                         (u16*)wp, R, Cc, ob, jd, oj1, oj2, flip, scale);
    else
      hipLaunchKernelGGL(pack_transpose_kernel<float>, grid, dim3(256), 0, as_stream(stream), w,
                         (float*)wp, R, Cc, ob, jd, oj1, oj2, flip, scale);
    return launch_status();
  }
  if (dtype == MMAD_BF16)
    hipLaunchKernelGGL(pack_weight_kernel<u16>, dim3(grid_for(total)), dim3(256), 0,
                       as_stream(stream), w, (u16*)wp, g.Nd, g.Kpad, g.K, g.Cs, g.cs_shift,
                       g.taps, mode, d->ci, d->kw, flip);
  else
    hipLaunchKernelGGL(pack_weight_kernel<float>, dim3(grid_for(total)), dim3(256), 0,
                       as_stream(stream), w, (float*)wp, g.Nd, g.Kpad, g.K, g.Cs, g.cs_shift,
                       g.taps, mode, d->ci, d->kw, flip);
  return launch_status();
}

int mmad_conv_pack_job(const mmad_conv_desc* d, int dtype, int for_dgrad, const float* w,
                       void* wp, int64_t tile0, mmad_pack_job* job) {
  if (!desc_ok(d)) return MMAD_EBADSHAPE;
  if (dtype != MMAD_F32 && dtype != MMAD_BF16) return MMAD_EBADDTYPE;
  if (!w || !wp || !job) return MMAD_ENULL;
  if (unfolded(d)) return MMAD_EUNSUPPORTED;
  const Geom g = for_dgrad ? dgrad_geom(d, dtype) : fwd_geom(d, dtype);
  if (!geom_ok(g, dtype) || g.Kpad != g.K) return MMAD_EUNSUPPORTED;
  const bool fw = !for_dgrad;
  mmad_pack_job j{};
  j.w = w;
  j.w_packed = wp;
  j.rows = fw ? d->co * d->ci : d->co;
  j.rdiv = fw ? d->ci : d->co;
  j.cols = fw ? g.taps : d->ci * g.taps;
  j.batch = 1;
  j.jdiv = g.taps;
  j.ostride_j2 = fw ? d->ci : d->co;
  j.ostride_b = fw ? g.Kpad : 0;
  j.ostride_j1 = fw ? 0 : g.Kpad;
  const bool narrow = j.cols <= 32;
  j.tiles_x = (int)cdiv(j.cols, narrow ? 32 : 64);
  j.tiles_y = (int)cdiv(j.rows, narrow ? 128 : 64);
  j.pad_ = for_dgrad && dgrad_as_fwd(d);
  j.tile0 = tile0;
  *job = j;
  return MMAD_OK;
}
// ... 443 lines not shown
```

multimodal_alzheimer_amd/csrc/patchconv.h:

```cpp
#pragma once
#include <stdint.h>

#include "../../include/mmad.h"

namespace mmad_patch {
struct Geo {
  int nb, Cs, Nd, Kpad;
  int Ds, Hs, Ws, Dd, Hd, Wd;
  int KD, KH, KW, pd, ph, pw, dd, dh, dw;
  const void* res = nullptr;
  int relu = 0;
  const void* bny = nullptr;
  const float* bnsc = nullptr;
  const float* bnsh = nullptr;
  const float* bnmu = nullptr;
  const float* bnis = nullptr;
  float* bnparts = nullptr;
};
bool ok(const Geo& g);
int64_t tiles(const Geo& g);
int fwd(const Geo& g, const void* src, const void* wp, const float* bias, void* dst,
        float* stats, void* stream);
}

namespace mmad_patchz {
int set_mode(int v);
bool ok(const mmad_patch::Geo& g);
int64_t tiles(const mmad_patch::Geo& g);
int fwd(const mmad_patch::Geo& g, const void* src, const void* wp, const float* bias, void* dst,
        float* stats, void* stream);
}

namespace mmad_lattice {
int set_mode(int v);
bool ok(const mmad_patch::Geo& g, int64_t fill_tiles);
int64_t tiles(const mmad_patch::Geo& g);
int fwd(const mmad_patch::Geo& g, const void* src, const void* wp, const float* bias, void* dst,
        float* stats, void* stream);
bool wgrad_ok(const mmad_patch::Geo& g);
int64_t wgrad_workspace(const mmad_patch::Geo& g);
int wgrad(const mmad_patch::Geo& g, const void* x, const void* dy, float* ws, int* splits,
          void* stream);
}

namespace mmad_s2 {
bool ok(const mmad_patch::Geo& g, int sd, int sh, int sw);
int64_t tiles(const mmad_patch::Geo& g);
int fwd(const mmad_patch::Geo& g, int sd, int sh, int sw, const void* src, const void* wp,
        const float* bias, void* dst, float* stats, void* stream);
bool dgrad_ok(const mmad_conv_desc* d);
int dgrad(const mmad_conv_desc* d, const void* dy, const void* wpt, void* dx, void* stream);
}

namespace mmad_lattice_zp {
int set_mode(int v);
bool ok(const mmad_patch::Geo& g);
int64_t tiles(const mmad_patch::Geo& g);
int fwd(const mmad_patch::Geo& g, const void* src, const void* wp, const float* bias, void* dst,
        float* stats, void* stream);
}

namespace mmad_lattice5 {
int set_mode(int v);
bool ok(const mmad_patch::Geo& g);
int64_t tiles(const mmad_patch::Geo& g);
int fwd(const mmad_patch::Geo& g, const void* src, const void* wp, const float* bias, void* dst,
        float* stats, void* stream);
bool wgrad_ok(const mmad_patch::Geo& g);
int64_t wgrad_workspace(const mmad_patch::Geo& g);
int wgrad(const mmad_patch::Geo& g, const void* x, const void* dy, float* ws, int* splits,
          void* stream);
}

namespace mmad_lattice8 {
int set_mode(int v);
bool ok(const mmad_patch::Geo& g);
int64_t tiles(const mmad_patch::Geo& g);
int fwd(const mmad_patch::Geo& g, const void* src, const void* wp, const float* bias, void* dst,
        float* stats, void* stream);
}

namespace mmad_pwgrad {
bool ok(const mmad_patch::Geo& g);
int64_t workspace(const mmad_patch::Geo& g);
int wgrad(const mmad_patch::Geo& g, const void* x, const void* dy, float* ws, int* splits,
          void* stream);
}

namespace mmad_pool {
int set_run_mode(int v);
}
```

multimodal_alzheimer_amd/csrc/pool.hip:

```cpp
#include <atomic>
#include <cstdlib>

#include "common.h"
#include "patchconv.h"

namespace {

struct PoolG {
  int n, c, di, hi, wi, do_, ho, wo, k, s, p;
};

template <typename T, int V>
__device__ __forceinline__ void load_v(const T* p, float* v) {
  if constexpr (V == Chunk<T>::N) Chunk<T>::load(p, v);
  else for (int e = 0; e < V; ++e) v[e] = Elt<T>::ld(p, e);
}
template <typename T, int V>
__device__ __forceinline__ void store_v(T* p, const float* v) {
  if constexpr (V == Chunk<T>::N) Chunk<T>::store(p, v);
  else for (int e = 0; e < V; ++e) Elt<T>::st(p, e, v[e]);
}

template <typename T, int V>
__global__ void maxpool_fwd_kernel(PoolG g, const T* __restrict__ x, T* __restrict__ y,
// ... 452 lines not shown
    const int ih = (int)(v % g.hi); v /= g.hi;
    const int id = (int)(v % g.di);
    const int64_t nb = v / g.di;
    auto lo = [&](int ii) { int q = ii + g.p - (g.k - 1); return q <= 0 ? 0 : (q + g.s - 1) / g.s; };
    auto hi = [&](int ii, int lim) { int q = (ii + g.p) / g.s; return q < lim - 1 ? q : lim - 1; };
    const int d0 = lo(id), d1 = hi(id, g.do_);
    const int h0 = lo(ih), h1 = hi(ih, g.ho);
    const int w0 = lo(iw), w1 = hi(iw, g.wo);
    float acc[V];
#pragma unroll
    for (int e = 0; e < V; ++e) acc[e] = 0.f;
    for (int od = d0; od <= d1; ++od)
      for (int oh = h0; oh <= h1; ++oh)
        for (int ow = w0; ow <= w1; ++ow) {
          const int wi = 0x80 | (((id - (od * g.s - g.p)) * g.k + (ih - (oh * g.s - g.p))) * g.k +
                                 (iw - (ow * g.s - g.p)));
          const int64_t o = (((nb * g.do_ + od) * g.ho + oh) * g.wo + ow) * g.c + c0;
          uint8_t a[V];
          if constexpr (V == 8) {
            const uint64_t w = *reinterpret_cast<const uint64_t*>(am + o);
#pragma unroll
            for (int e = 0; e < 8; ++e) a[e] = (uint8_t)(w >> (8 * e));
          } else if constexpr (V == 4) {
            const uint32_t w = *reinterpret_cast<const uint32_t*>(am + o);
#pragma unroll
            for (int e = 0; e < 4; ++e) a[e] = (uint8_t)(w >> (8 * e));
          } else {
            for (int e = 0; e < V; ++e) a[e] = am[o + e];
          }
          bool any = false;
#pragma unroll
          for (int e = 0; e < V; ++e) any |= a[e] == wi;
          if (!any) continue;
          float gv[V];
          load_v<T, V>(gp + o, gv);
#pragma unroll
          for (int e = 0; e < V; ++e)
            if (a[e] == wi) acc[e] += gv[e];
        }
    float yv[V], dv[V];
    load_v<T, V>(y + ivox * g.c + c0, yv);
#pragma unroll
    for (int e = 0; e < V; ++e) {
      const int c = c0 + e;
      const float xh = (yv[e] - mean[c]) * invstd[c];
      dv[e] = coef[c] * acc[e] - coef[g.c + c] - xh * coef[2 * g.c + c];
    }
    store_v<T, V>(dy + ivox * g.c + c0, dv);
  }
}

template <typename T, int V>
__global__ __launch_bounds__(1024) void gap_fwd_kernel(int64_t S, int C, int CB,
                                                      const T* __restrict__ x,
                                                      float* __restrict__ y) {
  __shared__ float red[1024 * 8];
  const int n = blockIdx.y;
  const int P = gridDim.z, part = blockIdx.z;
  const int64_t v0 = S * part / P, v1 = S * (part + 1) / P;
  const int cb0 = blockIdx.x * CB;
  const int cw = min(CB, C - cb0);
  const int lpr = cw / V;
  const int rpar = (int)blockDim.x / lpr;
  const int cl = threadIdx.x % lpr, rl = threadIdx.x / lpr;
  float s[V];
#pragma unroll
  for (int e = 0; e < V; ++e) s[e] = 0.f;
  if (rl < rpar) {
    for (int64_t v = v0 + rl; v < v1; v += rpar) {
      float val[V];
      load_v<T, V>(x + ((int64_t)n * S + v) * C + cb0 + cl * V, val);
#pragma unroll
      for (int e = 0; e < V; ++e) s[e] += val[e];
    }
#pragma unroll
    for (int e = 0; e < V; ++e) red[rl * cw + cl * V + e] = s[e];
  }
  __syncthreads();
  for (int c = threadIdx.x; c < cw; c += blockDim.x) {
    float acc = 0.f;
    for (int k = 0; k < rpar; ++k) acc += red[k * cw + c];
    if (P == 1) y[(int64_t)n * C + cb0 + c] = acc / (float)S;
    else y[((int64_t)n * P + part) * C + cb0 + c] = acc;
  }
}

__global__ void gap_fold_kernel(int n, int P, int C, int64_t S, const float* __restrict__ ws,
                                float* __restrict__ y) {
  const int64_t i = (int64_t)blockIdx.x * blockDim.x + threadIdx.x;
  if (i >= (int64_t)n * C) return;
  const int64_t b = i / C, c = i % C;
  float acc = 0.f;
#pragma unroll 16
  for (int p = 0; p < P; ++p) acc += ws[(b * P + p) * C + c];
  y[i] = acc / (float)S;
}

template <typename T, int V>
__global__ void gap_bwd_kernel(int n, int64_t S, int C, float inv, const float* __restrict__ dy,
                               T* __restrict__ dx) {
  const int cv = C / V;
  const int64_t total = (int64_t)n * S * cv;
  for (int64_t t = blockIdx.x * (int64_t)blockDim.x + threadIdx.x; t < total;
       t += (int64_t)gridDim.x * blockDim.x) {
    const int c0 = (int)(t % cv) * V;
    const int64_t nb = t / ((int64_t)S * cv);
    float v[V];
#pragma unroll
    for (int e = 0; e < V; ++e) v[e] = dy[nb * C + c0 + e] * inv;
    store_v<T, V>(dx + (t / cv) * C + c0, v);
  }
}

struct PlaneMax {
  uint32_t key[8], rb[8];
};
__device__ __forceinline__ void plane_max(const PoolG& g, __amdgpu_buffer_rsrc_t rs,
                                          uint32_t plane_off, const uint32_t (&wofs)[9], int y0,
                                          int x0, const f32x2* sc2, const f32x2* sh2,
                                          PlaneMax& m) {
#pragma unroll
  for (int e = 0; e < 8; ++e) { m.key[e] = 0; m.rb[e] = 0; }
  u32x4 raw[9];
  uint32_t tag[9];
#pragma unroll
  for (int w = 0; w < 9; ++w) {
    const int yc = min(max(y0 + w / 3, 0), g.hi - 1), xc = min(max(x0 + w % 3, 0), g.wi - 1);
    tag[w] = 31 - 18 - ((yc - y0) * 3 + (xc - x0));
    raw[w] = __builtin_bit_cast(u32x4, __builtin_amdgcn_raw_buffer_load_b128(
                                           rs, wofs[w], __builtin_amdgcn_readfirstlane(plane_off), 0));
  }
#pragma unroll
  for (int w = 0; w < 9; ++w) {
#pragma unroll
    for (int q = 0; q < 4; ++q) {
      const uint32_t word = raw[w][q];
      const f32x2 a = {__uint_as_float(word << 16), __uint_as_float(word & 0xffff0000u)};
      const f32x2 sv = __builtin_elementwise_fma(a, sc2[q], sh2[q]);
      const s16x2 v = __builtin_elementwise_max(
          __builtin_bit_cast(s16x2, __builtin_convertvector(sv, bf16x2)), (s16x2){0, 0});
      const uint32_t pk = __builtin_bit_cast(uint32_t, v);
      const uint32_t k0 = (pk << 16) | tag[w], k1 = (pk & 0xffff0000u) | tag[w];
      if (k0 > m.key[2 * q]) { m.key[2 * q] = k0; m.rb[2 * q] = word; }
      if (k1 > m.key[2 * q + 1]) { m.key[2 * q + 1] = k1; m.rb[2 * q + 1] = word; }
    }
  }
}
__device__ __forceinline__ void zmerge(PlaneMax& best, const PlaneMax& m, uint32_t add) {
#pragma unroll
  for (int e = 0; e < 8; ++e) {
    const uint32_t k = m.key[e] + add;
    if (k > best.key[e]) { best.key[e] = k; best.rb[e] = m.rb[e]; }
  }
}

#ifndef POOL_ZW_WAVES
#define POOL_ZW_WAVES 1
#endif
#ifndef POOL_ZW_ODS
#define POOL_ZW_ODS 4
#endif
__global__ __launch_bounds__(256, POOL_ZW_WAVES) void bnpool3s2_fwd_zwalk_kernel(
    PoolG g, int cv_shift, int ods, const u16* __restrict__ y, const float* __restrict__ scale,
    const float* __restrict__ shift, u16* __restrict__ out, uint8_t* __restrict__ am,
    u16* __restrict__ ymax) {
  const int cvn = 1 << cv_shift;
// ... 241 lines not shown
                       void* stream) {
  PoolG g{n, c, di, hi, wi, do_, ho, wo, k, s, p};
  if (!pool_ok(g)) return MMAD_EBADSHAPE;
  if (!dy || !dx || !argmax) return MMAD_ENULL;
  if (dtype == MMAD_BF16) return pool_bwd<u16>(g, dy, argmax, dx, as_stream(stream));
  if (dtype == MMAD_F32) return pool_bwd<float>(g, dy, argmax, dx, as_stream(stream));
  return MMAD_EBADDTYPE;
}

int mmad_bnpool_fwd(int dtype, int n, int c, int di, int hi, int wi, int do_, int ho, int wo,
                    int k, int s, int p, const void* y, const float* scale, const float* shift,
                    void* out, uint8_t* argmax, void* ymax, void* stream) {
  PoolG g{n, c, di, hi, wi, do_, ho, wo, k, s, p};
  if (!pool_ok(g) || k * k * k > 127) return MMAD_EBADSHAPE;
  if (!y || !scale || !shift || !out || !argmax || !ymax) return MMAD_ENULL;
  if (dtype == MMAD_BF16)
    return bnpool_fwd<u16>(g, y, scale, shift, out, argmax, ymax, as_stream(stream));
  if (dtype == MMAD_F32)
    return bnpool_fwd<float>(g, y, scale, shift, out, argmax, ymax, as_stream(stream));
  return MMAD_EBADDTYPE;
}

int mmad_bnpool_bwd_apply(int dtype, int n, int c, int di, int hi, int wi, int do_, int ho,
                          int wo, int k, int s, int p, const void* g, const uint8_t* argmax,
                          const void* y, const float* mean, const float* invstd,
                          const float* coef, void* dy, void* stream) {
  PoolG pg{n, c, di, hi, wi, do_, ho, wo, k, s, p};
  if (!pool_ok(pg) || k * k * k > 127) return MMAD_EBADSHAPE;
  if (!g || !argmax || !y || !mean || !invstd || !coef || !dy) return MMAD_ENULL;
  if (dtype == MMAD_BF16)
    return bnpool_bwd_apply<u16>(pg, g, argmax, y, mean, invstd, coef, dy, as_stream(stream));
  if (dtype == MMAD_F32)
    return bnpool_bwd_apply<float>(pg, g, argmax, y, mean, invstd, coef, dy, as_stream(stream));
  return MMAD_EBADDTYPE;
}

int mmad_gap_fwd(int dtype, int n, int64_t s, int c, const void* x, float* y, void* stream) {
  if (n <= 0 || s <= 0 || c <= 0) return MMAD_EBADSHAPE;
  if (!x || !y) return MMAD_ENULL;
  if (dtype == MMAD_BF16) return gap_fwd<u16>(n, s, c, x, y, as_stream(stream));
  if (dtype == MMAD_F32) return gap_fwd<float>(n, s, c, x, y, as_stream(stream));
  return MMAD_EBADDTYPE;
}

int64_t mmad_gap_fwd_ws_elems(int n, int64_t s, int c) {
  if (n <= 0 || s <= 0 || c <= 0) return -1;
  return (int64_t)n * gap_parts(n, s, c) * c;
}

int mmad_gap_fwd_ws(int dtype, int n, int64_t s, int c, const void* x, float* y, float* ws,
                    void* stream) {
  if (n <= 0 || s <= 0 || c <= 0) return MMAD_EBADSHAPE;
  if (!x || !y || !ws) return MMAD_ENULL;
  const int P = gap_parts(n, s, c);
  if (dtype == MMAD_BF16) return gap_fwd<u16>(n, s, c, x, y, as_stream(stream), ws, P);
  if (dtype == MMAD_F32) return gap_fwd<float>(n, s, c, x, y, as_stream(stream), ws, P);
  return MMAD_EBADDTYPE;
}

int mmad_gap_parts(int n, int64_t s, int c) {
  if (n <= 0 || s <= 0 || c <= 0) return -1;
  return gap_parts(n, s, c);
}

int mmad_gap_partial(int dtype, int n, int64_t s, int c, const void* x, float* ws,
                     void* stream) {
  if (n <= 0 || s <= 0 || c <= 0) return MMAD_EBADSHAPE;
  if (!x || !ws) return MMAD_ENULL;
  const int P = gap_parts(n, s, c);
  const int cb = std::min(c, 256);
  hipStream_t st = as_stream(stream);
  if (dtype == MMAD_BF16 && c % Chunk<u16>::N == 0 && cb % Chunk<u16>::N == 0)
    hipLaunchKernelGGL((gap_fwd_kernel<u16, Chunk<u16>::N>), dim3((unsigned)cdiv(c, cb),
                       (unsigned)n, (unsigned)P), dim3(1024), 0, st, s, c, cb, (const u16*)x, ws);
  else if (dtype == MMAD_F32 && c % Chunk<float>::N == 0 && cb % Chunk<float>::N == 0)
    hipLaunchKernelGGL((gap_fwd_kernel<float, Chunk<float>::N>), dim3((unsigned)cdiv(c, cb),
                       (unsigned)n, (unsigned)P), dim3(1024), 0, st, s, c, cb, (const float*)x,
                       ws);
  else
    return MMAD_EUNSUPPORTED;
  return launch_status();
}

int mmad_gap_bwd(int dtype, int n, int64_t s, int c, const float* dy, void* dx, void* stream) {
  if (n <= 0 || s <= 0 || c <= 0) return MMAD_EBADSHAPE;
  if (!dy || !dx) return MMAD_ENULL;
  if (dtype == MMAD_BF16) return gap_bwd<u16>(n, s, c, dy, dx, as_stream(stream));
  if (dtype == MMAD_F32) return gap_bwd<float>(n, s, c, dy, dx, as_stream(stream));
  return MMAD_EBADDTYPE;
}

int mmad_gap_bwd_compact(int dtype, int n, int64_t s, int c, const float* dy, void* dx,
                         void* stream) {
  if (n <= 0 || s <= 0 || c <= 0) return MMAD_EBADSHAPE;
  if (!dy || !dx) return MMAD_ENULL;
  if (dtype == MMAD_BF16) return gap_bwd<u16>(n, s, c, dy, dx, as_stream(stream), true);
  if (dtype == MMAD_F32) return gap_bwd<float>(n, s, c, dy, dx, as_stream(stream), true);
  return MMAD_EBADDTYPE;
}

}

namespace mmad_pool {
int set_run_mode(int v) {
  const int prev = pool_run_mode();
  if (v >= 0) g_pool_run.store(v, std::memory_order_relaxed);
  return prev;
}
}
```

multimodal_alzheimer_amd/head_ops.py:

```python
import ctypes as C

import torch

from . import _lib as L
from . import volume_ops as V
from .volume_ops import cast, grad_slot


class _LinearFn(torch.autograd.Function):
    @staticmethod
    def forward(ctx, x, weight, bias, relu):
        L.require_device(x, weight)
        if x.dtype != torch.float32:
            x = cast(x, torch.float32)
        x = x.contiguous()
        b, n_in = x.shape
        n_out = weight.shape[0]
        w = weight.detach().contiguous()
        bb = None if bias is None else bias.detach().contiguous()
        y = torch.empty((b, n_out), dtype=torch.float32, device=x.device)
        L.call("mmad_linear_fwd", b, n_in, n_out, L.ptr(x), L.ptr(w), L.ptr(bb), int(relu),
               L.ptr(y), L.stream())
        ctx.save_for_backward(x, weight, y if relu else None)
        ctx.has_bias = bias is not None
        ctx.relu = relu
        ctx.params = (weight, bias)
        return y

    @staticmethod
    def backward(ctx, g):
        x, weight, y = ctx.saved_tensors
        g = g.contiguous()
        if g.dtype != torch.float32:
            g = cast(g, torch.float32)
        b, n_in = x.shape
        n_out = weight.shape[0]
        dx = dw = db = None
        if ctx.needs_input_grad[0]:
            dx = torch.empty_like(x)
        need_w = ctx.needs_input_grad[1] or (ctx.has_bias and ctx.needs_input_grad[2])
        if need_w:
            dw = grad_slot(ctx.params[0], tuple(weight.shape), g.device)
            if ctx.has_bias:
                db = grad_slot(ctx.params[1], (n_out,), g.device)
        L.call("mmad_linear_bwd_ex", b, n_in, n_out, L.ptr(x), L.ptr(weight.detach()), L.ptr(g),
               L.ptr(y if ctx.relu else None), L.ptr(dx), L.ptr(dw), L.ptr(db), L.stream())
        return dx, (dw if ctx.needs_input_grad[1] else None), db, None


def linear(x, weight, bias=None, relu=False):
    return _LinearFn.apply(x, weight, bias, bool(relu))


class _GapLinearFn(torch.autograd.Function):

    @staticmethod
    def forward(ctx, x, weight, bias, relu):
        V._check_vol(x)
        lib = L.load()
        n, c = x.shape[:2]
        s = x.numel() // (n * c)
        parts = lib.mmad_gap_parts(n, s, c)
        ws = torch.empty(lib.mmad_gap_fwd_ws_elems(n, s, c), dtype=torch.float32,
                         device=x.device)
        L.call("mmad_gap_partial", L.dtype_code(x.dtype), n, s, c, L.ptr(x), L.ptr(ws),
               L.stream())
        n_out = weight.shape[0]
        w = weight.detach().contiguous()
        bb = None if bias is None else bias.detach().contiguous()
        xs = torch.empty((n, c), dtype=torch.float32, device=x.device)
        y = torch.empty((n, n_out), dtype=torch.float32, device=x.device)
        L.call("mmad_gap_linear_fwd", n, c, n_out, parts, s, L.ptr(ws), L.ptr(w), L.ptr(bb),
               int(relu), L.ptr(xs), L.ptr(y), L.stream())
        ctx.save_for_backward(xs, weight, y if relu else None)
        ctx.has_bias = bias is not None
        ctx.relu = relu
        ctx.params = (weight, bias)
        ctx.shape, ctx.dtype, ctx.s = tuple(x.shape), x.dtype, s
        return y

    @staticmethod
    def backward(ctx, g):
        xs, weight, y = ctx.saved_tensors
        g = g.contiguous()
        if g.dtype != torch.float32:
            g = cast(g, torch.float32)
        n, c = xs.shape
        n_out = weight.shape[0]
        rows = dw = db = None
        if ctx.needs_input_grad[0]:
            rows = torch.empty((n, c), dtype=ctx.dtype, device=g.device)
        if ctx.needs_input_grad[1] or (ctx.has_bias and ctx.needs_input_grad[2]):
            dw = grad_slot(ctx.params[0], tuple(weight.shape), g.device)
            if ctx.has_bias:
                db = grad_slot(ctx.params[1], (n_out,), g.device)
        L.call("mmad_linear_gap_bwd", n, c, n_out, ctx.s, L.ptr(xs), L.ptr(weight.detach()),
               L.ptr(g), L.ptr(y if ctx.relu else None), L.dtype_code(ctx.dtype), L.ptr(rows),
               L.ptr(dw), L.ptr(db), L.stream())
        dx = None if rows is None else rows.view(n, c, 1, 1, 1).expand(ctx.shape)
        return dx, (dw if ctx.needs_input_grad[1] else None), db, None


def gap_linear(x, weight, bias=None, relu=False):
    return _GapLinearFn.apply(x, weight, bias, bool(relu))


class _ConcatFn(torch.autograd.Function):
    @staticmethod
    def forward(ctx, *xs):
        L.require_device(*xs)
        xs = [x if x.dtype == torch.float32 else cast(x, torch.float32) for x in xs]
        xs = [x.contiguous() for x in xs]
        b = xs[0].shape[0]
        widths = [int(x.shape[1]) for x in xs]
        y = torch.empty((b, sum(widths)), dtype=torch.float32, device=xs[0].device)
        srcs = (C.c_void_p * len(xs))(*[x.data_ptr() for x in xs])
        ws = (C.c_int * len(xs))(*widths)
        L.call("mmad_concat_cols", b, len(xs), srcs, ws, L.ptr(y), L.stream())
        ctx.widths = widths
        return y

    @staticmethod
    def backward(ctx, g):
        g = g.contiguous()
        b = g.shape[0]
        outs = [torch.empty((b, w), dtype=torch.float32, device=g.device) for w in ctx.widths]
        dsts = (C.c_void_p * len(outs))(*[o.data_ptr() for o in outs])
        ws = (C.c_int * len(outs))(*ctx.widths)
        L.call("mmad_split_cols", b, len(outs), L.ptr(g), dsts, ws, L.stream())
        return tuple(outs)


def concat_features(*xs):
    if len(xs) > 8:
        raise L.MMADError("concat_features supports at most 8 inputs")
    return _ConcatFn.apply(*xs)


class _DropoutFn(torch.autograd.Function):
    @staticmethod
    def forward(ctx, x, p):
        L.require_device(x)
        dense = x.is_contiguous() or (x.dim() == 5 and
                                      x.is_contiguous(memory_format=torch.channels_last_3d))
        if not dense:
            x = x.contiguous()
        y = torch.empty_like(x)
        keep = torch.empty(x.numel(), dtype=torch.uint8, device=x.device)
        seed = torch.randint(0, 2 ** 62, (1,), dtype=torch.int64, device=x.device)
        L.call("mmad_dropout_fwd_dev", L.dtype_code(x.dtype), x.numel(), float(p), L.ptr(seed),
               L.ptr(x), L.ptr(y), L.ptr(keep), L.stream())
        ctx.save_for_backward(keep)
        ctx.p = p
        ctx.like = y
        return y

    @staticmethod
    def backward(ctx, g):
        (keep,) = ctx.saved_tensors
        g = g.contiguous(memory_format=torch.channels_last_3d) if g.dim() == 5 and \
            ctx.like.is_contiguous(memory_format=torch.channels_last_3d) else g.contiguous()
        dx = torch.empty_like(g)
        L.call("mmad_dropout_bwd", L.dtype_code(g.dtype), g.numel(), float(ctx.p), L.ptr(g),
               L.ptr(keep), L.ptr(dx), L.stream())
        return dx, None


def dropout(x, p, training):
    if not training or p == 0.0:
        return x
    if p >= 1.0:
        raise L.MMADError("dropout p must be < 1")
    return _DropoutFn.apply(x, float(p))


class _LossFn(torch.autograd.Function):
    @staticmethod
    def forward(ctx, logits, target, weight, gamma, mode):
        L.require_device(logits, target)
        x = logits.contiguous()
        if x.dtype != torch.float64:
            x = cast(x, torch.float64)
        t = target.contiguous().to(torch.int64) if target.dtype != torch.int64 else \
            target.contiguous()
        b, c = x.shape
        w = None if weight is None else weight.detach().to(torch.float64).contiguous()
# ... 91 lines not shown
```

multimodal_alzheimer_amd/layers.py:

```python
import os

import torch
import torch.nn as nn

from . import head_ops, volume_ops

_SUPPORTED_DTYPES = (torch.float32, torch.bfloat16)


def _triple(v):
    if isinstance(v, int):
        return (v, v, v)
    return tuple(int(a) for a in v)


class Conv3d(nn.Conv3d):

    compute_dtype = torch.float32

    def _pads(self):
        if isinstance(self.padding, str):
            if self.padding == "valid":
                return (0, 0, 0)
            pads = []
# ... 2 lines not shown
                    raise NotImplementedError("padding='same' with an even kernel extent")
                pads.append(d * (k - 1) // 2)
            return tuple(pads)
        return _triple(self.padding)

    _prepacked = None

    def _stride3(self):
        return _triple(self.stride)

    def _dilation3(self):
        return _triple(self.dilation)

    def forward_stats(self, x):
        return self._run(x, True)

    def _run(self, x, want_stats):
        if self.groups != 1 or self.padding_mode != "zeros":
            raise NotImplementedError("groups != 1 / non-zero padding_mode")
        cd = self.compute_dtype
        if isinstance(x, torch.Tensor) and x.shape[1] % 8 == 0 and x.dtype != cd:
            x = volume_ops.cast(x, cd)
        packed, self._prepacked = self._prepacked, None
        return volume_ops.conv3d(x, self.weight, self.bias, _triple(self.stride), self._pads(),
                                 _triple(self.dilation), cd, want_stats, packed)

    def forward(self, x):
        return self._run(x, False)


class BatchNorm3d(nn.BatchNorm3d):
    def forward(self, x):
        return volume_ops.batchnorm_act(x, self)


class BatchNorm1d(nn.BatchNorm1d):
    def forward(self, x):
        if x.dim() != 2:
            raise NotImplementedError("BatchNorm1d over (B, C, L) inputs")
        return volume_ops.batchnorm_act(x.contiguous(), self)


class ReLU(nn.ReLU):
    def forward(self, x):
        return volume_ops.relu(x)


class MaxPool3d(nn.MaxPool3d):
    def forward(self, x):
        k, s, p = _triple(self.kernel_size), _triple(self.stride or self.kernel_size), \
            _triple(self.padding)
        if len(set(k)) != 1 or len(set(s)) != 1 or len(set(p)) != 1 or \
                _triple(self.dilation) != (1, 1, 1) or self.ceil_mode or self.return_indices:
            raise NotImplementedError("MaxPool3d: cubic windows, dilation 1, floor mode only")
        return volume_ops.max_pool3d(x, k[0], s[0], p[0])


class AdaptiveAvgPool3d(nn.AdaptiveAvgPool3d):
    def forward(self, x):
        if _triple(self.output_size) != (1, 1, 1):
            raise NotImplementedError("AdaptiveAvgPool3d only to 1x1x1 (global average)")
        return volume_ops.global_avg_pool(x)


class Linear(nn.Linear):
    def forward(self, x):
        return head_ops.linear(x, self.weight, self.bias)


class Sequential(nn.Sequential):

    def forward(self, x):
        mods = list(self._modules.values())
        i = 0
        while i < len(mods):
            m = mods[i]
            nxt = mods[i + 1] if i + 1 < len(mods) else None
            k = _gap_linear_run(mods, i, x)
            if k:
                lin = mods[i + 2]
                x = head_ops.gap_linear(x, lin.weight, lin.bias, relu=k == 4)
                i += k
                continue
            if (type(m) is Linear and type(nxt) is ReLU and x.dim() == 2 and
                    not (m._forward_hooks or m._forward_pre_hooks or nxt._forward_hooks or
                         nxt._forward_pre_hooks)):
                x = head_ops.linear(x, m.weight, m.bias, relu=True)
                i += 2
                continue
            x = m(x)
            i += 1
        return x


GAP_LINEAR = os.environ.get("MMAD_GAP_LINEAR", "1") != "0"


def _gap_linear_run(mods, i, x):
    if not (GAP_LINEAR and volume_ops.GAP_BCAST) or i + 2 >= len(mods):
        return 0
    m, f, lin = mods[i], mods[i + 1], mods[i + 2]
    if not (type(m) is AdaptiveAvgPool3d and type(f) is nn.Flatten and type(lin) is Linear):
        return 0
    if lin.in_features > 4096:
        return 0
    if _triple(m.output_size) != (1, 1, 1) or f.start_dim != 1 or f.end_dim != -1:
        return 0
    if not (isinstance(x, torch.Tensor) and x.dim() == 5 and x.is_cuda and
            x.dtype in (torch.float32, torch.bfloat16)):
        return 0
    if x.shape[1] != lin.in_features:
        return 0
    relu =i + 3 < len(mods) and type(mods[i + 3]) is ReLU
    used = mods[i:i + (4 if relu else 3)]
    if any(u._forward_hooks or u._forward_pre_hooks for u in used):
        return 0
    return 4 if relu else 3


class Dropout(nn.Dropout):
    def forward(self, x):
        return head_ops.dropout(x, self.p, self.training)


class CrossEntropyLoss(nn.CrossEntropyLoss):

    def forward(self, input, target):
        if self.ignore_index != -100 or self.label_smoothing != 0.0 or self.reduction != "mean":
            raise NotImplementedError("only weighted 'mean' cross entropy")
        return head_ops.weighted_cross_entropy(input, target, self.weight)

    def fused_spec(self):
        if self.ignore_index != -100 or self.label_smoothing != 0.0 or self.reduction != "mean":
            return None
        return self.weight, 0.0, 0


_TORCH_TO_HIP = {
    nn.Conv3d: Conv3d, nn.BatchNorm3d: BatchNorm3d, nn.BatchNorm1d: BatchNorm1d,
    nn.ReLU: ReLU, nn.MaxPool3d: MaxPool3d, nn.AdaptiveAvgPool3d: AdaptiveAvgPool3d,
    nn.Linear: Linear, nn.Dropout: Dropout,
}


def set_compute_dtype(module, dtype):
    if dtype not in _SUPPORTED_DTYPES:
        raise ValueError(f"compute dtype must be one of {_SUPPORTED_DTYPES}")
    for m in module.modules():
        if isinstance(m, Conv3d):
            m.compute_dtype = dtype
    return module


def precision_dtype(hparams):
    p = str((hparams or {}).get("precision", "32")).lower()
    if p in ("32", "fp32", "float32", "32-true"):
        return torch.float32
    if p in ("bf16", "bfloat16", "bf16-mixed", "bf16-true"):
        return torch.bfloat16
    raise ValueError(f"unsupported precision {p!r}")
```

multimodal_alzheimer_amd/medicalnet.py:

```python
import argparse
import os

import torch
import torch.nn as nn

from . import layers as Lyr
from . import volume_ops as V

DEPTHS = {10: ("basic", (1, 1, 1, 1)), 18: ("basic", (2, 2, 2, 2)),
          34: ("basic", (3, 4, 6, 3)), 50: ("bottleneck", (3, 4, 6, 3))}
FEATURES = {10: 512, 18: 512, 34: 512, 50: 2048}


def _conv(cin, cout, k, stride=1, dilation=1):
    return Lyr.Conv3d(cin, cout, k, stride=stride, padding=dilation * (k // 2),
                      dilation=dilation, bias=False)


EVAL_FUSED = True


def _eval_fused_ok(block, x):
    return (EVAL_FUSED and not block.training and not torch.is_grad_enabled() and x.is_cuda
            and x.dim() == 5)


def _conv_bn_act(conv, bn, x, relu=True, res=None, res_conv=None, res_bn=None, res_x=None,
                 twin=False):
    y, parts = conv.forward_stats(x)
    if res_conv is not None:
        r, rparts = res_conv.forward_stats(res_x)
        return V.batchnorm_act(y, bn, parts, relu=relu, res=r, res_bn=res_bn, res_parts=rparts,
                               twin=twin)
    return V.batchnorm_act(y, bn, parts, relu=relu, res=res, twin=twin)




class BasicBlock(nn.Module):
    expansion = 1
    twin_out = False

    def __init__(self, cin, planes, stride=1, dilation=1, downsample=None):
        super().__init__()
        self.conv1 = _conv(cin, planes, 3, stride, dilation)
        self.bn1 = Lyr.BatchNorm3d(planes)
        self.relu = Lyr.ReLU(inplace=True)
        self.conv2 = _conv(planes, planes, 3, 1, dilation)
        self.bn2 = Lyr.BatchNorm3d(planes)
        self.downsample = downsample
        self.stride = stride
        self.dilation = dilation

    def forward(self, x):
        if _eval_fused_ok(self, x):
            y = self._eval_fused(x)
            if y is not None:
                return y
        h = _conv_bn_act(self.conv1, self.bn1, x)
        xr = V.take_twin(x)
        if self.downsample is None:
            return _conv_bn_act(self.conv2, self.bn2, h, res=xr, twin=self.twin_out)
        return _conv_bn_act(self.conv2, self.bn2, h, res_conv=self.downsample[0],
                            res_bn=self.downsample[1], res_x=xr, twin=self.twin_out)

    def _eval_fused(self, x):
        h = V.conv_bn_act_eval(x, self.conv1, self.bn1, relu=True)
        if h is None:
            return None
        if self.downsample is None:
            res = x if x.dtype == h.dtype else None
        else:
            res = V.conv_bn_act_eval(x, self.downsample[0], self.downsample[1], relu=False)
        if res is None:
            return None
        return V.conv_bn_act_eval(h, self.conv2, self.bn2, relu=True, res=res)


class Bottleneck(nn.Module):
    expansion = 4
    twin_out = False

    def __init__(self, cin, planes, stride=1, dilation=1, downsample=None):
        super().__init__()
        self.conv1 = _conv(cin, planes, 1)
        self.bn1 = Lyr.BatchNorm3d(planes)
        self.conv2 = _conv(planes, planes, 3, stride, dilation)
        self.bn2 = Lyr.BatchNorm3d(planes)
        self.conv3 = _conv(planes, planes * 4, 1)
        self.bn3 = Lyr.BatchNorm3d(planes * 4)
        self.relu = Lyr.ReLU(inplace=True)
        self.downsample = downsample
        self.stride = stride
        self.dilation = dilation

    def forward(self, x):
        h = _conv_bn_act(self.conv1, self.bn1, x)
        xr = V.take_twin(x)
        h = _conv_bn_act(self.conv2, self.bn2, h)
        if self.downsample is None:
            return _conv_bn_act(self.conv3, self.bn3, h, res=xr, twin=self.twin_out)
        return _conv_bn_act(self.conv3, self.bn3, h, res_conv=self.downsample[0],
                            res_bn=self.downsample[1], res_x=xr, twin=self.twin_out)


class ResNet(nn.Module):
    def __init__(self, depth=10, n_seg_classes=2, shortcut_type="B"):
        super().__init__()
        if depth not in DEPTHS:
            raise ValueError(f"resnet depth {depth} not in {sorted(DEPTHS)}")
        if shortcut_type != "B":
            raise NotImplementedError("only MedicalNet shortcut 'B' (the reference default)")
        kind, counts = DEPTHS[depth]
        block = BasicBlock if kind == "basic" else Bottleneck
        self.depth = depth
        self._cin = 64
        self.conv1 = Lyr.Conv3d(1, 64, 7, stride=2, padding=3, bias=False)
        self.bn1 = Lyr.BatchNorm3d(64)
        self.relu = Lyr.ReLU(inplace=True)
        self.maxpool = Lyr.MaxPool3d(3, stride=2, padding=1)
        self.layer1 = self._stage(block, 64, counts[0], 1, 1)
        self.layer2 = self._stage(block, 128, counts[1], 2, 1)
        self.layer3 = self._stage(block, 256, counts[2], 1, 2)
        self.layer4 = self._stage(block, 512, counts[3], 1, 4)
        blocks = [b for s in (self.layer1, self.layer2, self.layer3, self.layer4) for b in s]
        for b in blocks[:-1]:
            b.twin_out = True
        self.conv_seg = nn.Sequential(
            nn.ConvTranspose3d(512 * block.expansion, 32, 2, stride=2), nn.BatchNorm3d(32),
            nn.ReLU(inplace=True), nn.Conv3d(32, 32, 3, padding=1, bias=False),
            nn.BatchNorm3d(32), nn.ReLU(inplace=True),
            nn.Conv3d(32, n_seg_classes, 1, bias=False))
        for m in self.modules():
            if isinstance(m, nn.Conv3d):
                nn.init.kaiming_normal_(m.weight, mode="fan_out")
            elif isinstance(m, nn.BatchNorm3d):
                m.weight.data.fill_(1)
                m.bias.data.zero_()

    def _stage(self, block, planes, count, stride, dilation):
        ds = None
        if stride != 1 or self._cin != planes * block.expansion:
            ds = nn.Sequential(Lyr.Conv3d(self._cin, planes * block.expansion, 1, stride=stride,
                                          bias=False),
                               Lyr.BatchNorm3d(planes * block.expansion))
        blocks = [block(self._cin, planes, stride, dilation, ds)]
        self._cin = planes * block.expansion
        blocks += [block(self._cin, planes, 1, dilation) for _ in range(1, count)]
        return nn.Sequential(*blocks)

    def forward_features(self, x):
        if self.conv1.weight.is_cuda and not _eval_fused_ok(self, x):
            V.prepack(self)
        V.clear_twins()
        y, parts = self.conv1.forward_stats(x)
        mp = self.maxpool
        x = V.batchnorm_relu_maxpool(y, self.bn1, parts, mp.kernel_size, mp.stride, mp.padding,
                                     twin=True)
        return self.layer4(self.layer3(self.layer2(self.layer1(x))))

    def forward(self, x):
        return self.conv_seg(self.forward_features(x))


def resnet(depth, **kw):
    return ResNet(depth, **kw)


def parse_opts(argv=()):
    p = argparse.ArgumentParser(add_help=False)
    p.add_argument("--model", default="resnet")
    p.add_argument("--model_depth", type=int, default=10)
    p.add_argument("--resnet_shortcut", default="B")
    p.add_argument("--input_D", type=int, default=56)
    p.add_argument("--input_H", type=int, default=448)
    p.add_argument("--input_W", type=int, default=448)
    p.add_argument("--n_seg_classes", type=int, default=2)
    p.add_argument("--no_cuda", action="store_true")
    p.add_argument("--gpu_id", nargs="+", default=[0])
    p.add_argument("--pretrain_path", default="")
    p.add_argument("--phase", default="train")
    p.add_argument("--new_layer_names", default=["conv_seg"])
    return p.parse_args(list(argv))


def load_pretrained(net, path):
    ck = torch.load(path, map_location="cpu", weights_only=True)
    sd = ck.get("state_dict", ck)
    own = net.state_dict()
    sd = {k[len("module."):] if k.startswith("module.") else k: v for k, v in sd.items()}
    own.update({k: v for k, v in sd.items() if k in own and own[k].shape == v.shape})
    net.load_state_dict(own)


class _Wrapped(nn.Module):

    def __init__(self, m):
        super().__init__()
        self.module = m

    def forward(self, *a):
        return self.module(*a)


def generate_model(opts):
    net = ResNet(int(opts.model_depth), int(getattr(opts, "n_seg_classes", 2)),
                 getattr(opts, "resnet_shortcut", "B"))
    path = getattr(opts, "pretrain_path", "")
    if path and os.path.exists(path) and getattr(opts, "phase", "train") != "test":
        load_pretrained(net, path)
    return _Wrapped(net), net.parameters()
```

multimodal_alzheimer_amd/volume_ops.py:

```python
import ctypes as C
import os
import weakref

import torch

from . import _lib as L

CL = torch.channels_last_3d


def _cl(t):
    if t.dim() == 5:
        return t.contiguous(memory_format=CL)
    return t.contiguous()


def _empty_vol(n, c, d, h, w, dtype, device):
    return torch.empty((n, c, d, h, w), dtype=dtype, device=device, memory_format=CL)


def _check_vol(x, dtype=None):
    L.require_device(x)
    if x.dim() != 5 or not x.is_contiguous(memory_format=CL):
        raise L.MMADError("volume tensors must be 5-D channels_last_3d (NDHWC)")
# ... 683 lines not shown
_BNSUM_PARTS = {}


def _bnsum_source(x, d, dt):
    ent = _BNSUM_SRC.get(id(x))
    if ent is None or ent[0]() is not x:
        return None
    return ent[1] if L.load().mmad_conv3d_dgrad_bnsum_rows(d, dt) > 0 else None


def _bnsum_parts(g):
    ent = _BNSUM_PARTS.pop(id(g), None)
    return ent[1] if ent is not None and ent[0]() is g else None


def _sum_grads(g, g2):
    out = torch.empty_like(g)
    L.call("mmad_add", L.dtype_code(g.dtype), g.numel(), L.ptr(g), L.ptr(g2), L.ptr(out),
           L.stream())
    return out


def _twin_grads(g, g2, like):
    if g is None:
        g, g2 = g2, None
    out = []
    for t in (g, g2):
        if t is not None:
            t = _cl(t) if like.dim() == 5 else t.contiguous()
            if t.dtype != like.dtype:
                t = cast(t, like.dtype)
        out.append(t)
    return out


def _mask_from_y_ok(y):
    c = y.shape[1]
    v = 8 if y.dtype == torch.bfloat16 else 4
    return c % v == 0 and (c // v) & (c // v - 1) == 0 and c // v <= 256


def _bn_backward(g, relu_out, y, mean, invstd, gamma, batch_stats, want_gmask,
                 params=(None, None), mask_affine=None, g2=None, pre_parts=None):
    m, c = _rows(y)
    dev = y.device
    dt = L.dtype_code(y.dtype)
    if g2 is not None and (mask_affine is not None or not _mask_from_y_ok(y)):
        g, g2 = _sum_grads(g, g2), None
    if pre_parts is not None:
        parts = pre_parts
        nparts = parts.shape[0]
    else:
        nparts = L.load().mmad_bn_bwd_parts(m, c)
        parts = torch.empty((nparts, 2, c), dtype=torch.float32, device=dev)
    if pre_parts is not None:
        pass
    elif mask_affine is not None:
        sc, sh = mask_affine
        L.call("mmad_bn_relu_bwd_reduce", dt, m, c, L.ptr(g), L.ptr(y), L.ptr(mean),
               L.ptr(invstd), L.ptr(sc), L.ptr(sh), L.ptr(parts), L.stream())
    else:
        L.call("mmad_bn_bwd_reduce", dt, m, c, L.ptr(g), L.ptr(g2), L.ptr(relu_out), L.ptr(y),
               L.ptr(mean), L.ptr(invstd), L.ptr(parts), L.stream())
    dgamma = grad_slot(params[0], (c,), dev)
    dbeta = grad_slot(params[1], (c,), dev)
    coef = torch.empty(3 * c, dtype=torch.float32, device=dev)
    L.call("mmad_bn_bwd_finalize", c, m, nparts, L.ptr(parts), L.ptr(gamma), L.ptr(invstd),
           int(batch_stats), L.ptr(dgamma), L.ptr(dbeta), L.ptr(coef), L.stream())
    dy = torch.empty_like(y)
    gmask = torch.empty_like(y) if want_gmask else None
    if mask_affine is not None:
        L.call("mmad_bn_relu_bwd_apply", dt, m, c, L.ptr(g), L.ptr(y), L.ptr(mean),
               L.ptr(invstd), L.ptr(mask_affine[0]), L.ptr(mask_affine[1]), L.ptr(coef),
               L.ptr(dy), L.stream())
    else:
        L.call("mmad_bn_bwd_apply", dt, m, c, L.ptr(g), L.ptr(g2), L.ptr(relu_out), L.ptr(y),
               L.ptr(mean), L.ptr(invstd), L.ptr(coef), L.ptr(dy), L.ptr(gmask), L.stream())
    return dy, dgamma, dbeta, gmask


_BN_DUAL = os.environ.get("MMAD_BN_DUAL", "1") != "0"


def _bn_backward_pair(g, relu_out, y, mean, invstd, gamma, batch_stats, y2, mean2, invstd2,
                      gamma2, batch_stats2, params, params2, g2=None, g_rows=0):
    m, c = _rows(y)
    dev = y.device
    dt = L.dtype_code(y.dtype)
    nparts = L.load().mmad_bn_bwd_parts(m, c)
    parts = torch.empty((2, nparts, 2, c), dtype=torch.float32, device=dev)
    L.call("mmad_bn_bwd_reduce2", dt, m, c, L.ptr(g), L.ptr(g2), g_rows, L.ptr(relu_out),
           L.ptr(y), L.ptr(mean), L.ptr(invstd), L.ptr(y2), L.ptr(mean2), L.ptr(invstd2),
           L.ptr(parts[0]), L.ptr(parts[1]), L.stream())
    dgamma = grad_slot(params[0], (c,), dev)
    dbeta = grad_slot(params[1], (c,), dev)
    dgamma2 = grad_slot(params2[0], (c,), dev)
    dbeta2 = grad_slot(params2[1], (c,), dev)
    coef = torch.empty((2, 3 * c), dtype=torch.float32, device=dev)
    L.call("mmad_bn_bwd_finalize2", c, m, nparts, L.ptr(parts[0]), L.ptr(gamma), L.ptr(invstd),
           int(batch_stats), L.ptr(dgamma), L.ptr(dbeta), L.ptr(coef[0]), L.ptr(parts[1]),
           L.ptr(gamma2), L.ptr(invstd2), int(batch_stats2), L.ptr(dgamma2), L.ptr(dbeta2),
           L.ptr(coef[1]), L.stream())
    dy = torch.empty_like(y)
    dy2 = torch.empty_like(y2)
    L.call("mmad_bn_bwd_apply2", dt, m, c, L.ptr(g), L.ptr(g2), g_rows, L.ptr(relu_out),
           L.ptr(y), L.ptr(mean), L.ptr(invstd), L.ptr(coef[0]), L.ptr(dy), L.ptr(y2),
           L.ptr(mean2), L.ptr(invstd2), L.ptr(coef[1]), L.ptr(dy2), L.stream())
    return dy, dgamma, dbeta, dy2, dgamma2, dbeta2


class _BNActFn(torch.autograd.Function):

    @staticmethod
    def forward(ctx, y, parts, gamma, beta, res, res_parts, rgamma, rbeta, cfg):
        bn, relu, training, rbn, twin, bnsum = cfg
        L.require_device(y)
        rscale = rshift = rmean = rinvstd = None
        rbatch = False
        if rbn is not None and _BN_DUAL:
            (mean, invstd, scale, shift, batch), (rmean, rinvstd, rscale, rshift, rbatch) = \
                _finalize_pair(y, parts, bn, res, res_parts, rbn, training)
        else:
            mean, invstd, scale, shift, batch = _finalize(y, parts, bn, training)
            if rbn is not None:
                rmean, rinvstd, rscale, rshift, rbatch = _finalize(res, res_parts, rbn, training)
        out = torch.empty_like(y)
        m, c = _rows(y)
        L.call("mmad_scale_shift_act", L.dtype_code(y.dtype), m, c, L.ptr(y), L.ptr(scale),
               L.ptr(shift), L.ptr(res), L.ptr(rscale), L.ptr(rshift), int(relu), L.ptr(out),
               L.stream())
        masky = relu and res is None and y.dim() == 5 and _mask_from_y_ok(y)
        if masky and bnsum and not twin and y.dtype == torch.bfloat16:
            _BNSUM_SRC[id(out)] = (weakref.ref(out), (y, mean, invstd, scale, shift))
        ctx.save_for_backward(y, out if relu and not masky else None, mean, invstd, gamma,
                              res if rbn is not None else None, rmean, rinvstd, rgamma)
        ctx.mask_affine = (scale, shift) if masky else None
        ctx.cfg = (relu, batch, rbatch, res is not None, rbn is not None)
        ctx.params = ((gamma, beta), (rgamma, rbeta))
        if twin:
            ctx.set_materialize_grads(False)
            return out, out.view(out.shape)
        return out

    @staticmethod
    def backward(ctx, g, g2=None):
        y, out, mean, invstd, gamma, rres, rmean, rinvstd, rgamma = ctx.saved_tensors
        relu, batch, rbatch, has_res, has_rbn = ctx.cfg
        pair = (has_rbn and _BN_DUAL and out is not None and ctx.mask_affine is None
                and _mask_from_y_ok(y))
        g_rows = _gap_rows(g, y) if pair and y.numel() // y.shape[1] < 2 ** 31 else 0
        if g_rows:
            g2 = _twin_grads(g2, None, y)[0]
        else:
            g, g2 = _twin_grads(g, g2, y)
        if g is None:
            return (None,) * 9
        gam = None if gamma is None else gamma.detach()
        if pair:
            rg = None if rgamma is None else rgamma.detach()
            dy, dgamma, dbeta, dres, drg, drb = _bn_backward_pair(
                g, out, y, mean, invstd, gam, batch, rres, rmean, rinvstd, rg, rbatch,
                ctx.params[0], ctx.params[1], g2, g_rows)
            return (dy, None, dgamma if ctx.needs_input_grad[2] else None,
                    dbeta if ctx.needs_input_grad[3] else None, dres, None,
                    drg if ctx.needs_input_grad[6] else None,
                    drb if ctx.needs_input_grad[7] else None, None)
        if g2 is not None and has_rbn:
            g, g2 = _sum_grads(g, g2), None
        pre = _bnsum_parts(g) if ctx.mask_affine is not None and g2 is None and \
            _BNSUM_PARTS else None
        dy, dgamma, dbeta, gmask = _bn_backward(g, out, y, mean, invstd, gam, batch,
                                                has_res and not has_rbn, ctx.params[0],
                                                ctx.mask_affine, g2, pre)
        dres = drg = drb = None
        if has_rbn:
            rg = None if rgamma is None else rgamma.detach()
            dres, drg, drb, _ = _bn_backward(g, out, rres, rmean, rinvstd, rg, rbatch, False,
                                             ctx.params[1])
        elif has_res:
            dres = gmask
        return (dy, None, dgamma if ctx.needs_input_grad[2] else None,
                dbeta if ctx.needs_input_grad[3] else None, dres, None,
                drg if ctx.needs_input_grad[6] else None,
                drb if ctx.needs_input_grad[7] else None, None)


def batchnorm_act(y, bn, parts=None, relu=False, res=None, res_bn=None, res_parts=None,
                  twin=False):
    if y.dim() == 5:
        _check_vol(y)
    elif not y.is_contiguous():
        raise L.MMADError("batchnorm_act expects a contiguous (B, C) tensor")
    if res is not None:
        if res.shape != y.shape or res.dtype != y.dtype:
            raise L.MMADError("residual must match the BN input in shape and dtype")
        if y.dim() == 5:
            _check_vol(res)
    training = bn.training or not bn.track_running_stats
    twin = _twin_wanted(twin, y)
    out = _BNActFn.apply(y, parts, bn.weight, bn.bias, res, res_parts,
                         None if res_bn is None else res_bn.weight,
                         None if res_bn is None else res_bn.bias,
                         (bn, relu, training, res_bn, twin,
                          BNSUM and torch.is_grad_enabled()))
    if twin:
        out, alias = out
        _register_twin(out, alias)
    return out


class _BNReluPoolFn(torch.autograd.Function):

    @staticmethod
    def forward(ctx, y, parts, gamma, beta, cfg):
        bn, training, k, s, p, twin = cfg
        mean, invstd, scale, shift, batch = _finalize(y, parts, bn, training)
        n, c, di, hi, wi = y.shape
        do, ho, wo = ((v + 2 * p - k) // s + 1 for v in (di, hi, wi))
        out = _empty_vol(n, c, do, ho, wo, y.dtype, y.device)
        ymax = torch.empty_like(out)
        am = torch.empty((n, do, ho, wo, c), dtype=torch.uint8, device=y.device)
        L.call("mmad_bnpool_fwd", L.dtype_code(y.dtype), n, c, di, hi, wi, do, ho, wo, k, s, p,
               L.ptr(y), L.ptr(scale), L.ptr(shift), L.ptr(out), L.ptr(am), L.ptr(ymax),
               L.stream())
        ctx.save_for_backward(y, am, ymax, mean, invstd, gamma)
        ctx.params = (gamma, beta)
        ctx.geo = (n, c, di, hi, wi, do, ho, wo, k, s, p)
        ctx.batch = batch
        if twin:
            ctx.set_materialize_grads(False)
            return out, out.view(out.shape)
        return out

    @staticmethod
    def backward(ctx, g, g2=None):
        y, am, ymax, mean, invstd, gamma = ctx.saved_tensors
        n, c, di, hi, wi, do, ho, wo, k, s, p = ctx.geo
        g, g2 = _twin_grads(g, g2, y)
        if g is None:
            return (None,) * 5
        dt = L.dtype_code(y.dtype)
        dev = y.device
        mp = n * do * ho * wo
        nparts = L.load().mmad_bn_bwd_parts(mp, c)
        parts = torch.empty((nparts, 2, c), dtype=torch.float32, device=dev)
# ... 232 lines not shown
```

Baseline: 2805 volumes/sec.

## Recompute relu mask from BN pair affine and fuse tail BN-act into GAP

For the BN-plus-BN-residual relu output, backward now recomputes the relu mask from y, y2 and the saved scale/shift pairs instead of saving and reloading the output tensor. This removes one activation-sized read per pass and lets the output be freed early. The last ResNet block's BN+residual+relu is deferred: a fused kernel computes the activation and global-average-pool partial sums directly, skipping the write and re-read of the final activation. Both paths sit behind environment switches and add kernel variants and a lazy DeferredTail object, which risks hook and shape-compatibility edge cases.

```diff
diff --git a/include/mmad.h b/include/mmad.h
--- a/include/mmad.h
+++ b/include/mmad.h
@@ -177,6 +177,19 @@
                        int64_t g_rows, const void* relu_out, const void* y, const float* mean, const float* invstd, const float* coef,
                        void* dy, const void* y2, const float* mean2, const float* invstd2,
                        const float* coef2, void* dy2, void* stream);
+int mmad_bn_bwd_reduce2_affine(int dtype, int64_t m, int c, const void* g, const void* g2,
+                               int64_t g_rows, const float* scale, const float* shift,
+                               const float* rscale, const float* rshift, const void* y,
+                               const float* mean, const float* invstd, const void* y2,
+                               const float* mean2, const float* invstd2, float* parts,
+                               float* parts2, void* stream);
+int mmad_bn_bwd_apply2_affine(int dtype, int64_t m, int c, const void* g, const void* g2,
+                              int64_t g_rows, const float* scale, const float* shift,
+                              const float* rscale, const float* rshift, const void* y,
+                              const float* mean, const float* invstd, const float* coef,
+                              void* dy, const void* y2, const float* mean2,
+                              const float* invstd2, const float* coef2, void* dy2,
+                              void* stream);
 int mmad_bn_relu_bwd_reduce(int dtype, int64_t m, int c, const void* g, const void* y,
                             const float* mean, const float* invstd, const float* scale,
                             const float* shift, float* parts, void* stream);
@@ -215,6 +228,9 @@
 int mmad_gap_parts(int n, int64_t s, int c);
 int mmad_gap_partial(int dtype, int n, int64_t s, int c, const void* x, float* ws,
                      void* stream);
+int mmad_bn_act_gap_partial(int dtype, int n, int64_t s, int c, const void* y,
+                            const float* scale, const float* shift, const void* y2,
+                            const float* rscale, const float* rshift, float* ws, void* stream);
 int mmad_gap_linear_fwd(int b, int in, int out, int parts, int64_t s, const float* ws,
                         const float* w, const float* bias, int relu, float* xs, float* y,
                         void* stream);
diff --git a/multimodal_alzheimer_amd/_lib.py b/multimodal_alzheimer_amd/_lib.py
--- a/multimodal_alzheimer_amd/_lib.py
+++ b/multimodal_alzheimer_amd/_lib.py
@@ -125,6 +125,8 @@
     "mmad_bn_bwd_finalize2": (_i32, [_i32, _i64, _i32, _vp, _vp, _vp, _i32, _vp, _vp, _vp,
                                      _vp, _vp, _vp, _i32, _vp, _vp, _vp, _vp]),
     "mmad_bn_bwd_apply2": (_i32, [_i32, _i64, _i32, _vp, _vp, _i64] + [_vp] * 12),
+    "mmad_bn_bwd_reduce2_affine": (_i32, [_i32, _i64, _i32, _vp, _vp, _i64] + [_vp] * 13),
+    "mmad_bn_bwd_apply2_affine": (_i32, [_i32, _i64, _i32, _vp, _vp, _i64] + [_vp] * 15),
     "mmad_relu_fwd": (_i32, [_i32, _i64, _vp, _vp, _vp]),
     "mmad_relu_bwd": (_i32, [_i32, _i64, _vp, _vp, _vp, _vp]),
     "mmad_colsum_ws": (_i32, [_i32, _i64, _i32, _vp, _vp, _vp, _vp]),
@@ -148,6 +150,7 @@
     "mmad_gap_bwd_compact": (_i32, [_i32, _i32, _i64, _i32, _vp, _vp, _vp]),
     "mmad_gap_parts": (_i32, [_i32, _i64, _i32]),
     "mmad_gap_partial": (_i32, [_i32, _i32, _i64, _i32, _vp, _vp, _vp]),
+    "mmad_bn_act_gap_partial": (_i32, [_i32, _i32, _i64, _i32] + [_vp] * 8),
     "mmad_gap_linear_fwd": (_i32, [_i32, _i32, _i32, _i32, _i64, _vp, _vp, _vp, _i32, _vp,
                                    _vp, _vp]),
     "mmad_linear_gap_bwd": (_i32, [_i32, _i32, _i32, _i64, _vp, _vp, _vp, _vp, _i32, _vp, _vp,
diff --git a/multimodal_alzheimer_amd/csrc/bn.hip b/multimodal_alzheimer_amd/csrc/bn.hip
--- a/multimodal_alzheimer_amd/csrc/bn.hip
+++ b/multimodal_alzheimer_amd/csrc/bn.hip
@@ -1,4 +1,9 @@
+#include <atomic>
+#include <cstdlib>
+#include <type_traits>
+
 #include "common.h"
+#include "patchconv.h"
 
 constexpr int COLSUM_ROWS = 4;
 
@@ -22,7 +27,8 @@
 __device__ float g_fold_sink[4096];
 #endif
 
-template <typename T, int MODE, int V, bool DUAL = false, bool G2 = false, bool GB = false>
+template <typename T, int MODE, int V, bool DUAL = false, bool G2 = false, bool GB = false,
+          bool PM = false>
 __global__ __launch_bounds__(256) void colsum_kernel(int64_t M, int C, int64_t rpp,
                                                      const T* __restrict__ y,
                                                      const T* __restrict__ g,
@@ -39,8 +45,11 @@
                                                      float* __restrict__ parts2 = nullptr,
                                                      const T* __restrict__ g2 = nullptr,
                                                      T* __restrict__ gsum = nullptr,
-                                                     uint32_t gS = 0) {
+                                                     uint32_t gS = 0,
+                                                     const float* __restrict__ rsc = nullptr,
+                                                     const float* __restrict__ rsh = nullptr) {
   static_assert(!DUAL || MODE == 1, "dual partial sums: BN backward with a relu_out mask");
+  static_assert(!PM || DUAL, "mask from the inputs: the pair kernel");
   static_assert(!GB || (DUAL && V == Chunk<T>::N), "broadcast g: the pair kernel, 16-byte rows");
   __shared__ float red[DUAL ? 3 : 2][2048];
   const int tid = threadIdx.x;
@@ -55,7 +64,7 @@
 #pragma unroll
   for (int e = 0; e < V; ++e) { s[e] = 0.f; q[e] = 0.f; q2[e] = 0.f; }
   if (rl < rpar) {
-    float mu[V], is[V], sc[V], sh[V], mu2[V], is2[V];
+    float mu[V], is[V], sc[V], sh[V], mu2[V], is2[V], rs[V], rh[V];
     if (MODE == 1 || MODE == 3 || MODE == 4) {
 #pragma unroll
       for (int e = 0; e < V; ++e) { mu[e] = mean[cb + cl * V + e]; is[e] = invstd[cb + cl * V + e]; }
@@ -67,10 +76,15 @@
         is2[e] = invstd2[cb + cl * V + e];
       }
     }
-    if (MODE == 4) {
+    if (MODE == 4 || PM) {
 #pragma unroll
       for (int e = 0; e < V; ++e) { sc[e] = msc[cb + cl * V + e]; sh[e] = msh[cb + cl * V + e]; }
     }
+    if constexpr (PM) {
+#pragma unroll
+      for (int e = 0; e < V; ++e) { rs[e] = rsc[cb + cl * V + e]; rh[e] = rsh[cb + cl * V + e]; }
+    }
+    const bool ld_out = !PM && MODE == 1 && relu_out != nullptr;
     auto accum = [&](int64_t i, float* yv, float* gv, const float* ov, const float* y2v) {
       if (MODE == 1 || MODE == 3 || MODE == 4) {
         if (MODE == 4) {
@@ -79,6 +93,10 @@
         } else if (MODE == 3) {
 #pragma unroll
           for (int e = 0; e < V; ++e) gv[e] = (act[i + e] & 0x80) ? gv[e] : 0.f;
+        } else if constexpr (PM) {
+#pragma unroll
+          for (int e = 0; e < V; ++e)
+            gv[e] = pair_out<T>(yv[e], sc[e], sh[e], y2v[e], rs[e], rh[e]) > 0.f ? gv[e] : 0.f;
         } else if (relu_out != nullptr) {
 #pragma unroll
           for (int e = 0; e < V; ++e) gv[e] = ov[e] > 0.f ? gv[e] : 0.f;
@@ -116,8 +134,7 @@
           else if (NEED_G)
             gr[u] = *reinterpret_cast<const u32x4*>(g + i);
           if (NEED_G && G2) g2r[u] = *reinterpret_cast<const u32x4*>(g2 + i);
-          if (MODE == 1 && relu_out != nullptr)
-            orr[u] = *reinterpret_cast<const u32x4*>(relu_out + i);
+          if (ld_out) orr[u] = *reinterpret_cast<const u32x4*>(relu_out + i);
           if constexpr (DUAL) y2r[u] = *reinterpret_cast<const u32x4*>(y2 + i);
         }
 #pragma unroll
@@ -133,8 +150,7 @@
             for (int e = 0; e < V; ++e) gv[e] = as_stored<T>(gv[e] + hv[e]);
             if constexpr (MODE == 3) Chunk<T>::store(gsum + i, gv);
           }
-          if (MODE == 1 && relu_out != nullptr)
-            Chunk<T>::load(reinterpret_cast<const T*>(&orr[u]), ov);
+          if (ld_out) Chunk<T>::load(reinterpret_cast<const T*>(&orr[u]), ov);
           if constexpr (DUAL) Chunk<T>::load(reinterpret_cast<const T*>(&y2r[u]), y2v);
           accum(i, yv, gv, ov, y2v);
         }
@@ -160,7 +176,7 @@
             else for (int e = 0; e < V; ++e) Elt<T>::st(gsum, i + e, gv[e]);
           }
         }
-        if (MODE == 1 && relu_out != nullptr) {
+        if (ld_out) {
           if constexpr (V == Chunk<T>::N) Chunk<T>::load(relu_out + i, ov);
           else for (int e = 0; e < V; ++e) ov[e] = Elt<T>::ld(relu_out, i + e);
         }
@@ -464,9 +480,10 @@
 #pragma unroll
     for (int e = 0; e < N; ++e) {
       const int c = c0 + e;
-      float o = bn_affine(v[e], scale[c], shift[c]);
+      float o;
+      if (RES == 2) o = pair_sum(v[e], scale[c], shift[c], r[e], rscale[c], rshift[c]);
+      else o = bn_affine(v[e], scale[c], shift[c]);
       if (RES == 1) o += r[e];
-      if (RES == 2) o += r[e] * rscale[c] + rshift[c];
       v[e] = relu ? fmaxf(o, 0.f) : o;
     }
     Chunk<T>::store(out + i0, v);
@@ -501,9 +518,10 @@
   auto apply = [&](float* v, const float* r) {
 #pragma unroll
     for (int e = 0; e < N; ++e) {
-      float o = bn_affine(v[e], sc[e], sh[e]);
+      float o;
+      if (RES == 2) o = pair_sum(v[e], sc[e], sh[e], r[e], rs[e], rh[e]);
+      else o = bn_affine(v[e], sc[e], sh[e]);
       if (RES == 1) o += r[e];
-      if (RES == 2) o += r[e] * rs[e] + rh[e];
       v[e] = relu ? fmaxf(o, 0.f) : o;
     }
   };
@@ -542,8 +560,13 @@
   for (int64_t i = blockIdx.x * (int64_t)blockDim.x + threadIdx.x; i < n;
        i += (int64_t)gridDim.x * blockDim.x) {
     const int c = (int)(i % C);
-    float o = bn_affine(Elt<T>::ld(y, i), scale[c], shift[c]);
-    if (res) o += rscale ? Elt<T>::ld(res, i) * rscale[c] + rshift[c] : Elt<T>::ld(res, i);
+    float o;
+    if (res && rscale)
+      o = pair_sum(Elt<T>::ld(y, i), scale[c], shift[c], Elt<T>::ld(res, i), rscale[c],
+                   rshift[c]);
+    else
+      o = bn_affine(Elt<T>::ld(y, i), scale[c], shift[c]);
+    if (res && !rscale) o += Elt<T>::ld(res, i);
     Elt<T>::st(out, i, relu ? fmaxf(o, 0.f) : o);
   }
 }
@@ -554,16 +577,22 @@
   const float* invstd2;
   const float* coef2;
   void* dy2;
+  const float* rsc;
+  const float* rsh;
 };
 
-template <typename T, bool MASKY = false, bool DUAL = false, bool G2 = false, bool GB = false>
-__global__ __launch_bounds__(256) void bn_bwd_apply_fc_kernel(
+template <typename T, bool MASKY = false, bool DUAL = false, bool G2 = false, bool GB = false,
+          bool PM = false>
+__global__ __launch_bounds__(256)
+__attribute__((amdgpu_waves_per_eu(PM && GB ? 2 : 1, PM && GB ? 2 : 8)))
+void bn_bwd_apply_fc_kernel(
     int64_t nv, int cpr, int C, const T* __restrict__ g, const T* __restrict__ relu_out,
     const T* __restrict__ y, const float* __restrict__ mean, const float* __restrict__ invstd,
     const float* __restrict__ coef, T* __restrict__ dy, T* __restrict__ gmask,
     const float* __restrict__ msc = nullptr, const float* __restrict__ msh = nullptr,
     BwdApply2 d2 = {}, const T* __restrict__ g2 = nullptr, uint32_t gS = 0) {
   constexpr int V = Chunk<T>::N;
+  static_assert(!PM || (DUAL && !MASKY), "mask from the inputs: the pair kernel");
   const int cpr_shift = __builtin_ctz(cpr);
   auto g_at = [&](int64_t qq) -> const T* {
     if constexpr (GB)
@@ -581,13 +610,18 @@
   ld_params<V>(coef + C + c0, k1);
   ld_params<V>(coef + 2 * C + c0, k2);
   float sc[V], sh[V];
-  if constexpr (MASKY) {
+  if constexpr (MASKY || PM) {
     ld_params<V>(msc + c0, sc);
     ld_params<V>(msh + c0, sh);
   }
   const T* __restrict__ y2 = static_cast<const T*>(d2.y2);
   T* __restrict__ dy2 = static_cast<T*>(d2.dy2);
-  float mu2[V], is2[V], j0[V], j1[V], j2[V];
+  float mu2[V], is2[V], j0[V], j1[V], j2[V], rs[V], rh[V];
+  if constexpr (PM) {
+    ld_params<V>(d2.rsc + c0, rs);
+    ld_params<V>(d2.rsh + c0, rh);
+  }
+  const bool ld_out = !PM && relu_out != nullptr;
   if constexpr (DUAL) {
     ld_params<V>(d2.mean2 + c0, mu2);
     ld_params<V>(d2.invstd2 + c0, is2);
@@ -600,8 +634,12 @@
     float gv[V], dv[V], dv2[V];
 #pragma unroll
     for (int e = 0; e < V; ++e) {
-      if constexpr (MASKY) gv[e] = bn_affine(yv[e], sc[e], sh[e]) > 0.f ? gv0[e] : 0.f;
-      else gv[e] = (relu_out && !(ov[e] > 0.f)) ? 0.f : gv0[e];
+      if constexpr (MASKY)
+        gv[e] = bn_affine(yv[e], sc[e], sh[e]) > 0.f ? gv0[e] : 0.f;
+      else if constexpr (PM)
+        gv[e] = pair_out<T>(yv[e], sc[e], sh[e], y2v[e], rs[e], rh[e]) > 0.f ? gv0[e] : 0.f;
+      else
+        gv[e] = (relu_out && !(ov[e] > 0.f)) ? 0.f : gv0[e];
       const float xh = (yv[e] - mu[e]) * is[e];
       dv[e] = k0[e] * gv[e] - k1[e] - xh * k2[e];
       if constexpr (DUAL) {
@@ -630,7 +668,7 @@
     }
     Chunk<T>::load(y + q * V, y0);
     Chunk<T>::load(y + (q + stride) * V, y1);
-    if (relu_out) {
+    if (ld_out) {
       Chunk<T>::load(relu_out + q * V, o0);
       Chunk<T>::load(relu_out + (q + stride) * V, o1);
     }
@@ -646,7 +684,7 @@
     Chunk<T>::load(g_at(q), g0);
     if constexpr (G2) add_g2(q, g0);
     Chunk<T>::load(y + q * V, y0);
-    if (relu_out) Chunk<T>::load(relu_out + q * V, o0);
+    if (ld_out) Chunk<T>::load(relu_out + q * V, o0);
     if constexpr (DUAL) Chunk<T>::load(y2 + q * V, z0);
     one(q, g0, y0, o0, z0);
   }
@@ -726,6 +764,33 @@
 
 bool dt_ok(int dtype) { return dtype == MMAD_F32 || dtype == MMAD_BF16; }
 
+struct Switch {
+  const char* env;
+  std::atomic<int> v{-1};
+  int get() {
+    int cur = v.load(std::memory_order_relaxed);
+    if (cur < 0) {
+      const char* e = getenv(env);
+      int expect = -1;
+      v.compare_exchange_strong(expect, e ? (atoi(e) != 0) : 1);
+      cur = v.load(std::memory_order_relaxed);
+    }
+    return cur;
+  }
+  int set(int nv) {
+    const int prev = get();
+    if (nv >= 0) v.store(nv, std::memory_order_relaxed);
+    return prev;
+  }
+};
+Switch g_pair_mask{"MMAD_PAIR_MASK"};
+Switch g_tail_gap{"MMAD_TAIL_GAP"};
+
+}
+
+namespace mmad_bn {
+int set_pair_mask(int v) { return g_pair_mask.set(v); }
+int set_tail_gap(int v) { return g_tail_gap.set(v); }
 }
 
 extern "C" {
@@ -966,15 +1031,26 @@
   return launch_status();
 }
 
-int mmad_bn_bwd_reduce2(int dtype, int64_t m, int c, const void* g, const void* g2,
-                        int64_t g_rows, const void* relu_out, const void* y, const float* mean,
-                        const float* invstd, const void* y2,
-                        const float* mean2, const float* invstd2, float* parts, float* parts2,
-                        void* stream) {
+}
+
+namespace {
+
+struct PairAffine {
+  const float* scale;
+  const float* shift;
+  const float* rscale;
+  const float* rshift;
+};
+
+int bn_bwd_reduce2(int dtype, int64_t m, int c, const void* g, const void* g2, int64_t g_rows,
+                   const void* relu_out, const PairAffine* aff, const void* y,
+                   const float* mean, const float* invstd, const void* y2, const float* mean2,
+                   const float* invstd2, float* parts, float* parts2, void* stream) {
   if (!dt_ok(dtype)) return MMAD_EBADDTYPE;
   if (m <= 0 || c <= 0) return MMAD_EBADSHAPE;
-  if (!g || !relu_out || !y || !mean || !invstd || !y2 || !mean2 || !invstd2 || !parts ||
-      !parts2)
+  if (!g || !y || !mean || !invstd || !y2 || !mean2 || !invstd2 || !parts || !parts2)
+    return MMAD_ENULL;
+  if (aff ? (!aff->scale || !aff->shift || !aff->rscale || !aff->rshift) : !relu_out)
     return MMAD_ENULL;
   if (g_rows < 0 || (g_rows > 0 && (m % g_rows || m >= (int64_t(1) << 31))))
     return MMAD_EBADSHAPE;
@@ -986,17 +1062,47 @@
     int slabs = 1;
     while (c % (slabs * 2 * VEC) == 0 && c / (slabs * VEC) > 256) slabs *= 2;
     if (!(c % (slabs * VEC) == 0 && c / (slabs * VEC) <= 256)) return MMAD_EUNSUPPORTED;
-    auto k = g_rows > 0 ? (g2 != nullptr ? colsum_kernel<T, 1, VEC, true, true, true>
-                                          : colsum_kernel<T, 1, VEC, true, false, true>)
-                        : (g2 != nullptr ? colsum_kernel<T, 1, VEC, true, true>
-                                          : colsum_kernel<T, 1, VEC, true, false>);
+    auto pick = [&](auto pm) {
+      constexpr bool PM = decltype(pm)::value;
+      return g_rows > 0 ? (g2 != nullptr ? colsum_kernel<T, 1, VEC, true, true, true, PM>
+                                         : colsum_kernel<T, 1, VEC, true, false, true, PM>)
+                        : (g2 != nullptr ? colsum_kernel<T, 1, VEC, true, true, false, PM>
+                                         : colsum_kernel<T, 1, VEC, true, false, false, PM>);
+    };
+    auto k = aff ? pick(std::true_type{}) : pick(std::false_type{});
     hipLaunchKernelGGL(k, dim3((unsigned)pp.nparts, slabs), dim3(256), 0, st, m, c, pp.rpp,
                        (const T*)y, (const T*)g, (const T*)relu_out, mean, invstd, parts,
-                       nullptr, nullptr, nullptr, (const T*)y2, mean2, invstd2, parts2,
-                       (const T*)g2, (T*)nullptr, (uint32_t)g_rows);
+                       nullptr, aff ? aff->scale : nullptr, aff ? aff->shift : nullptr,
+                       (const T*)y2, mean2, invstd2, parts2, (const T*)g2, (T*)nullptr,
+                       (uint32_t)g_rows, aff ? aff->rscale : nullptr,
+                       aff ? aff->rshift : nullptr);
     return launch_status();
   };
   return dtype == MMAD_BF16 ? go(u16{}) : go(float{});
+}
+
+}
+
+extern "C" {
+
+int mmad_bn_bwd_reduce2(int dtype, int64_t m, int c, const void* g, const void* g2,
+                        int64_t g_rows, const void* relu_out, const void* y, const float* mean,
+                        const float* invstd, const void* y2,
+                        const float* mean2, const float* invstd2, float* parts, float* parts2,
+                        void* stream) {
+  return bn_bwd_reduce2(dtype, m, c, g, g2, g_rows, relu_out, nullptr, y, mean, invstd, y2,
+                        mean2, invstd2, parts, parts2, stream);
+}
+
+int mmad_bn_bwd_reduce2_affine(int dtype, int64_t m, int c, const void* g, const void* g2,
+                               int64_t g_rows, const float* scale, const float* shift,
+                               const float* rscale, const float* rshift, const void* y,
+                               const float* mean, const float* invstd, const void* y2,
+                               const float* mean2, const float* invstd2, float* parts,
+                               float* parts2, void* stream) {
+  const PairAffine aff{scale, shift, rscale, rshift};
+  return bn_bwd_reduce2(dtype, m, c, g, g2, g_rows, nullptr, &aff, y, mean, invstd, y2, mean2,
+                        invstd2, parts, parts2, stream);
 }
 
 int mmad_bn_bwd_finalize2(int c, int64_t count, int nparts, const float* parts,
@@ -1013,30 +1119,44 @@
   return launch_status();
 }
 
-int mmad_bn_bwd_apply2(int dtype, int64_t m, int c, const void* g, const void* g2,
-                       int64_t g_rows, const void* relu_out, const void* y, const float* mean, const float* invstd, const float* coef,
-                       void* dy, const void* y2, const float* mean2, const float* invstd2,
-                       const float* coef2, void* dy2, void* stream) {
+}
+
+namespace {
+
+int bn_bwd_apply2(int dtype, int64_t m, int c, const void* g, const void* g2, int64_t g_rows,
+                  const void* relu_out, const PairAffine* aff, const void* y, const float* mean,
+                  const float* invstd, const float* coef, void* dy, const void* y2,
+                  const float* mean2, const float* invstd2, const float* coef2, void* dy2,
+                  void* stream) {
   if (!dt_ok(dtype)) return MMAD_EBADDTYPE;
   if (m <= 0 || c <= 0) return MMAD_EBADSHAPE;
-  if (!g || !relu_out || !y || !mean || !invstd || !coef || !dy || !y2 || !mean2 || !invstd2 ||
-      !coef2 || !dy2)
+  if (!g || !y || !mean || !invstd || !coef || !dy || !y2 || !mean2 || !invstd2 || !coef2 ||
+      !dy2)
+    return MMAD_ENULL;
+  if (aff ? (!aff->scale || !aff->shift || !aff->rscale || !aff->rshift) : !relu_out)
     return MMAD_ENULL;
   const int vv = dtype == MMAD_BF16 ? 8 : 4;
   if (!(c % vv == 0 && is_pow2(c / vv) && c / vv <= 256)) return MMAD_EUNSUPPORTED;
   const int64_t nv = m * c / vv;
-  const BwdApply2 d2{y2, mean2, invstd2, coef2, dy2};
+  const BwdApply2 d2{y2, mean2, invstd2, coef2, dy2, aff ? aff->rscale : nullptr,
+                     aff ? aff->rshift : nullptr};
+  const float* msc = aff ? aff->scale : nullptr;
+  const float* msh = aff ? aff->shift : nullptr;
   hipStream_t st = as_stream(stream);
   if (g_rows < 0 || (g_rows > 0 && (m % g_rows || m >= (int64_t(1) << 31))))
     return MMAD_EBADSHAPE;
-#define APPLY2(T, G, B)                                                                      \
-  hipLaunchKernelGGL((bn_bwd_apply_fc_kernel<T, false, true, G, B>), dim3(ew_grid(nv)),       \
+#define APPLY2(T, G, B, PM)                                                                  \
+  hipLaunchKernelGGL((bn_bwd_apply_fc_kernel<T, false, true, G, B, PM>), dim3(ew_grid(nv)),   \
                      dim3(256), 0, st, nv, c / vv, c, (const T*)g, (const T*)relu_out,        \
-                     (const T*)y, mean, invstd, coef, (T*)dy, (T*)nullptr, nullptr, nullptr,  \
-                     d2, (const T*)g2, (uint32_t)g_rows)
+                     (const T*)y, mean, invstd, coef, (T*)dy, (T*)nullptr, msc, msh, d2,      \
+                     (const T*)g2, (uint32_t)g_rows)
 #define APPLY2G(T, B)                                                                        \
   do {                                                                                       \
-    if (g2 != nullptr) APPLY2(T, true, B); else APPLY2(T, false, B);                         \
+    if (aff) {                                                                               \
+      if (g2 != nullptr) APPLY2(T, true, B, true); else APPLY2(T, false, B, true);           \
+    } else {                                                                                 \
+      if (g2 != nullptr) APPLY2(T, true, B, false); else APPLY2(T, false, B, false);         \
+    }                                                                                        \
   } while (0)
   if (dtype == MMAD_BF16) {
     if (g_rows > 0) APPLY2G(u16, true); else APPLY2G(u16, false);
@@ -1046,6 +1166,31 @@
 #undef APPLY2G
 #undef APPLY2
   return launch_status();
+}
+
+}
+
+extern "C" {
+
+int mmad_bn_bwd_apply2(int dtype, int64_t m, int c, const void* g, const void* g2,
+                       int64_t g_rows, const void* relu_out, const void* y, const float* mean,
+                       const float* invstd, const float* coef, void* dy, const void* y2,
+                       const float* mean2, const float* invstd2, const float* coef2, void* dy2,
+                       void* stream) {
+  return bn_bwd_apply2(dtype, m, c, g, g2, g_rows, relu_out, nullptr, y, mean, invstd, coef, dy,
+                       y2, mean2, invstd2, coef2, dy2, stream);
+}
+
+int mmad_bn_bwd_apply2_affine(int dtype, int64_t m, int c, const void* g, const void* g2,
+                              int64_t g_rows, const float* scale, const float* shift,
+                              const float* rscale, const float* rshift, const void* y,
+                              const float* mean, const float* invstd, const float* coef,
+                              void* dy, const void* y2, const float* mean2,
+                              const float* invstd2, const float* coef2, void* dy2,
+                              void* stream) {
+  const PairAffine aff{scale, shift, rscale, rshift};
+  return bn_bwd_apply2(dtype, m, c, g, g2, g_rows, nullptr, &aff, y, mean, invstd, coef, dy, y2,
+                       mean2, invstd2, coef2, dy2, stream);
 }
 
 int mmad_relu_bwd(int dtype, int64_t n, const void* g, const void* out, void* dx, void* stream) {
diff --git a/multimodal_alzheimer_amd/csrc/common.h b/multimodal_alzheimer_amd/csrc/common.h
--- a/multimodal_alzheimer_amd/csrc/common.h
+++ b/multimodal_alzheimer_amd/csrc/common.h
@@ -122,6 +122,18 @@
   else return v;
 }
 
+__device__ __forceinline__ float pair_sum(float y, float scale, float shift, float res,
+                                          float rscale, float rshift) {
+  float o = bn_affine(y, scale, shift);
+  o += res * rscale + rshift;
+  return o;
+}
+template <typename T>
+__device__ __forceinline__ float pair_out(float y, float scale, float shift, float res,
+                                          float rscale, float rshift) {
+  return as_stored<T>(pair_sum(y, scale, shift, res, rscale, rshift));
+}
+
 __device__ __forceinline__ float wave_sum(float v) {
 #pragma unroll
   for (int o = 32; o > 0; o >>= 1) v += __shfl_xor(v, o, 64);
diff --git a/multimodal_alzheimer_amd/csrc/conv.hip b/multimodal_alzheimer_amd/csrc/conv.hip
--- a/multimodal_alzheimer_amd/csrc/conv.hip
+++ b/multimodal_alzheimer_amd/csrc/conv.hip
@@ -1452,6 +1452,8 @@
   if (std::strcmp(name, "pool_run") == 0) return mmad_pool::set_run_mode(value);
   if (std::strcmp(name, "patchz") == 0) return mmad_patchz::set_mode(value);
   if (std::strcmp(name, "pw_wg3_dedup") == 0) return mmad_pw::set_wg3_dedup(value);
+  if (std::strcmp(name, "pair_mask") == 0) return mmad_bn::set_pair_mask(value);
+  if (std::strcmp(name, "tail_gap") == 0) return mmad_bn::set_tail_gap(value);
   return -1;
 }
 
diff --git a/multimodal_alzheimer_amd/csrc/patchconv.h b/multimodal_alzheimer_amd/csrc/patchconv.h
--- a/multimodal_alzheimer_amd/csrc/patchconv.h
+++ b/multimodal_alzheimer_amd/csrc/patchconv.h
@@ -90,3 +90,8 @@
 namespace mmad_pool {
 int set_run_mode(int v);
 }
+
+namespace mmad_bn {
+int set_pair_mask(int v);
+int set_tail_gap(int v);
+}
diff --git a/multimodal_alzheimer_amd/csrc/pool.hip b/multimodal_alzheimer_amd/csrc/pool.hip
--- a/multimodal_alzheimer_amd/csrc/pool.hip
+++ b/multimodal_alzheimer_amd/csrc/pool.hip
@@ -558,6 +558,69 @@
     for (int k = 0; k < rpar; ++k) acc += red[k * cw + c];
     if (P == 1) y[(int64_t)n * C + cb0 + c] = acc / (float)S;
     else y[((int64_t)n * P + part) * C + cb0 + c] = acc;
+  }
+}
+
+template <typename T>
+__global__ __launch_bounds__(1024, 8) void bn_act_gap_kernel(
+    int64_t S, int C, int CB, const T* __restrict__ y, const T* __restrict__ y2,
+    const float* __restrict__ scale, const float* __restrict__ shift,
+    const float* __restrict__ rscale, const float* __restrict__ rshift, float* __restrict__ ws) {
+  constexpr int V = Chunk<T>::N;
+  __shared__ float red[1024 * 8];
+  const int n = blockIdx.y;
+  const int P = gridDim.z, part = blockIdx.z;
+  const int64_t v0 = S * part / P, v1 = S * (part + 1) / P;
+  const int cb0 = blockIdx.x * CB;
+  const int cw = min(CB, C - cb0);
+  const int lpr = cw / V;
+  const int rpar = (int)blockDim.x / lpr;
+  const int cl = threadIdx.x % lpr, rl = threadIdx.x / lpr;
+  float s[V];
+#pragma unroll
+  for (int e = 0; e < V; ++e) s[e] = 0.f;
+  if (rl < rpar) {
+    float sc[V], sh[V], rs[V], rh[V];
+#pragma unroll
+    for (int e = 0; e < V; e += 4) {
+      const int c = cb0 + cl * V + e;
+      const f32x4 a = *reinterpret_cast<const f32x4*>(scale + c);
+      const f32x4 b = *reinterpret_cast<const f32x4*>(shift + c);
+      const f32x4 d = *reinterpret_cast<const f32x4*>(rscale + c);
+      const f32x4 f = *reinterpret_cast<const f32x4*>(rshift + c);
+#pragma unroll
+      for (int k = 0; k < 4; ++k) { sc[e + k] = a[k]; sh[e + k] = b[k]; rs[e + k] = d[k]; rh[e + k] = f[k]; }
+    }
+    auto add_row = [&](const u32x4& ar, const u32x4& br) {
+#pragma unroll
+      for (int k = 0; k < 4; ++k) {
+        if constexpr (sizeof(T) == 2) {
+          const float a0 = __uint_as_float(ar[k] << 16), b0 = __uint_as_float(br[k] << 16);
+          const float a1 = __uint_as_float(ar[k] & 0xffff0000u);
+          const float b1 = __uint_as_float(br[k] & 0xffff0000u);
+          const int e = 2 * k;
+          s[e] += as_stored<T>(fmaxf(pair_sum(a0, sc[e], sh[e], b0, rs[e], rh[e]), 0.f));
+          s[e + 1] += as_stored<T>(
+              fmaxf(pair_sum(a1, sc[e + 1], sh[e + 1], b1, rs[e + 1], rh[e + 1]), 0.f));
+        } else {
+          s[k] += fmaxf(pair_sum(__uint_as_float(ar[k]), sc[k], sh[k], __uint_as_float(br[k]),
+                                 rs[k], rh[k]), 0.f);
+        }
+      }
+    };
+    for (int64_t v = v0 + rl; v < v1; v += rpar) {
+      const int64_t i = ((int64_t)n * S + v) * C + cb0 + cl * V;
+      add_row(*reinterpret_cast<const u32x4*>(y + i), *reinterpret_cast<const u32x4*>(y2 + i));
+    }
+#pragma unroll
+    for (int e = 0; e < V; ++e) red[rl * cw + cl * V + e] = s[e];
+  }
+  __syncthreads();
+  for (int c = threadIdx.x; c < cw; c += blockDim.x) {
+    float acc = 0.f;
+    for (int k = 0; k < rpar; ++k) acc += red[k * cw + c];
+    if (P == 1) ws[(int64_t)n * C + cb0 + c] = acc / (float)S;
+    else ws[((int64_t)n * P + part) * C + cb0 + c] = acc;
   }
 }
 
@@ -965,6 +1028,27 @@
   return launch_status();
 }
 
+int mmad_bn_act_gap_partial(int dtype, int n, int64_t s, int c, const void* y,
+                            const float* scale, const float* shift, const void* y2,
+                            const float* rscale, const float* rshift, float* ws,
+                            void* stream) {
+  if (n <= 0 || s <= 0 || c <= 0) return MMAD_EBADSHAPE;
+  if (!y || !scale || !shift || !y2 || !rscale || !rshift || !ws) return MMAD_ENULL;
+  const int P = gap_parts(n, s, c);
+  const int cb = std::min(c, 256);
+  hipStream_t st = as_stream(stream);
+  const dim3 grid((unsigned)cdiv(c, cb), (unsigned)n, (unsigned)P);
+  if (dtype == MMAD_BF16 && c % Chunk<u16>::N == 0 && cb % Chunk<u16>::N == 0)
+    hipLaunchKernelGGL(bn_act_gap_kernel<u16>, grid, dim3(1024), 0, st, s, c, cb,
+                       (const u16*)y, (const u16*)y2, scale, shift, rscale, rshift, ws);
+  else if (dtype == MMAD_F32 && c % Chunk<float>::N == 0 && cb % Chunk<float>::N == 0)
+    hipLaunchKernelGGL(bn_act_gap_kernel<float>, grid, dim3(1024), 0, st, s, c, cb,
+                       (const float*)y, (const float*)y2, scale, shift, rscale, rshift, ws);
+  else
+    return MMAD_EUNSUPPORTED;
+  return launch_status();
+}
+
 int mmad_gap_bwd(int dtype, int n, int64_t s, int c, const float* dy, void* dx, void* stream) {
   if (n <= 0 || s <= 0 || c <= 0) return MMAD_EBADSHAPE;
   if (!dy || !dx) return MMAD_ENULL;
diff --git a/multimodal_alzheimer_amd/head_ops.py b/multimodal_alzheimer_amd/head_ops.py
--- a/multimodal_alzheimer_amd/head_ops.py
+++ b/multimodal_alzheimer_amd/head_ops.py
@@ -101,7 +101,76 @@
         return dx, (dw if ctx.needs_input_grad[1] else None), db, None
 
 
+class _TailGapLinearFn(torch.autograd.Function):
+
+    @staticmethod
+    def forward(ctx, y, parts, gamma, beta, res, res_parts, rgamma, rbeta, weight, bias, cfg):
+        bn, rbn, relu = cfg
+        V._check_vol(y)
+        V._check_vol(res)
+        lib = L.load()
+        (mean, invstd, scale, shift, batch), (rmean, rinvstd, rscale, rshift, rbatch) = \
+            V._finalize_pair(y, parts, bn, res, res_parts, rbn, True)
+        n, c = y.shape[:2]
+        s = y.numel() // (n * c)
+        nparts = lib.mmad_gap_parts(n, s, c)
+        ws = torch.empty(lib.mmad_gap_fwd_ws_elems(n, s, c), dtype=torch.float32,
+                         device=y.device)
+        L.call("mmad_bn_act_gap_partial", L.dtype_code(y.dtype), n, s, c, L.ptr(y),
+               L.ptr(scale), L.ptr(shift), L.ptr(res), L.ptr(rscale), L.ptr(rshift), L.ptr(ws),
+               L.stream())
+        n_out = weight.shape[0]
+        w = weight.detach().contiguous()
+        bb = None if bias is None else bias.detach().contiguous()
+        xs = torch.empty((n, c), dtype=torch.float32, device=y.device)
+        out = torch.empty((n, n_out), dtype=torch.float32, device=y.device)
+        L.call("mmad_gap_linear_fwd", n, c, n_out, nparts, s, L.ptr(ws), L.ptr(w), L.ptr(bb),
+               int(relu), L.ptr(xs), L.ptr(out), L.stream())
+        ctx.save_for_backward(y, res, mean, invstd, gamma, rmean, rinvstd, rgamma, scale, shift,
+                              rscale, rshift, xs, weight, out if relu else None)
+        ctx.has_bias = bias is not None
+        ctx.relu = relu
+        ctx.batch = (batch, rbatch)
+        ctx.params = (weight, bias)
+        ctx.bn_params = ((gamma, beta), (rgamma, rbeta))
+        ctx.s = s
+        return out
+
+    @staticmethod
+    def backward(ctx, g):
+        (y, res, mean, invstd, gamma, rmean, rinvstd, rgamma, scale, shift, rscale, rshift, xs,
+         weight, out) = ctx.saved_tensors
+        g = g.contiguous()
+        if g.dtype != torch.float32:
+            g = cast(g, torch.float32)
+        n, c = xs.shape
+        n_out = weight.shape[0]
+        dw = db = None
+        rows = torch.empty((n, c), dtype=y.dtype, device=g.device)
+        if ctx.needs_input_grad[8] or (ctx.has_bias and ctx.needs_input_grad[9]):
+            dw = grad_slot(ctx.params[0], tuple(weight.shape), g.device)
+            if ctx.has_bias:
+                db = grad_slot(ctx.params[1], (n_out,), g.device)
+        L.call("mmad_linear_gap_bwd", n, c, n_out, ctx.s, L.ptr(xs), L.ptr(weight.detach()),
+               L.ptr(g), L.ptr(out if ctx.relu else None), L.dtype_code(y.dtype), L.ptr(rows),
+               L.ptr(dw), L.ptr(db), L.stream())
+        gam = None if gamma is None else gamma.detach()
+        rg = None if rgamma is None else rgamma.detach()
+        dy, dgamma, dbeta, dres, drg, drb = V._bn_backward_pair(
+            rows, None, y, mean, invstd, gam, ctx.batch[0], res, rmean, rinvstd, rg,
+            ctx.batch[1], ctx.bn_params[0], ctx.bn_params[1], None, ctx.s,
+            (scale, shift, rscale, rshift))
+        need = ctx.needs_input_grad
+        return (dy, None, dgamma if need[2] else None, dbeta if need[3] else None, dres, None,
+                drg if need[6] else None, drb if need[7] else None,
+                dw if need[8] else None, db, None)
+
+
 def gap_linear(x, weight, bias=None, relu=False):
+    if isinstance(x, V.DeferredTail):
+        bn, rbn = x.bn, x.res_bn
+        return _TailGapLinearFn.apply(x.y, x.parts, bn.weight, bn.bias, x.res, x.res_parts,
+                                      rbn.weight, rbn.bias, weight, bias, (bn, rbn, bool(relu)))
     return _GapLinearFn.apply(x, weight, bias, bool(relu))
 
 
diff --git a/multimodal_alzheimer_amd/layers.py b/multimodal_alzheimer_amd/layers.py
--- a/multimodal_alzheimer_amd/layers.py
+++ b/multimodal_alzheimer_amd/layers.py
@@ -108,6 +108,7 @@
                 x = head_ops.gap_linear(x, lin.weight, lin.bias, relu=k == 4)
                 i += k
                 continue
+            x = volume_ops.materialize(x)
             if (type(m) is Linear and type(nxt) is ReLU and x.dim() == 2 and
                     not (m._forward_hooks or m._forward_pre_hooks or nxt._forward_hooks or
                          nxt._forward_pre_hooks)):
@@ -116,7 +117,7 @@
                 continue
             x = m(x)
             i += 1
-        return x
+        return volume_ops.materialize(x)
 
 
 GAP_LINEAR = os.environ.get("MMAD_GAP_LINEAR", "1") != "0"
@@ -132,12 +133,13 @@
         return 0
     if _triple(m.output_size) != (1, 1, 1) or f.start_dim != 1 or f.end_dim != -1:
         return 0
-    if not (isinstance(x, torch.Tensor) and x.dim() == 5 and x.is_cuda and
+    if not (isinstance(x, (torch.Tensor, volume_ops.DeferredTail)) and x.dim() == 5 and
+            x.is_cuda and
             x.dtype in (torch.float32, torch.bfloat16)):
         return 0
     if x.shape[1] != lin.in_features:
         return 0
-    relu =i + 3 < len(mods) and type(mods[i + 3]) is ReLU
+    relu = i + 3 < len(mods) and type(mods[i + 3]) is ReLU
     used = mods[i:i + (4 if relu else 3)]
     if any(u._forward_hooks or u._forward_pre_hooks for u in used):
         return 0
diff --git a/multimodal_alzheimer_amd/medicalnet.py b/multimodal_alzheimer_amd/medicalnet.py
--- a/multimodal_alzheimer_amd/medicalnet.py
+++ b/multimodal_alzheimer_amd/medicalnet.py
@@ -40,6 +40,7 @@
 class BasicBlock(nn.Module):
     expansion = 1
     twin_out = False
+    defer_tail = False
 
     def __init__(self, cin, planes, stride=1, dilation=1, downsample=None):
         super().__init__()
@@ -61,6 +62,14 @@
         xr = V.take_twin(x)
         if self.downsample is None:
             return _conv_bn_act(self.conv2, self.bn2, h, res=xr, twin=self.twin_out)
+        if self.defer_tail and not self.twin_out:
+            y, parts = self.conv2.forward_stats(h)
+            r, rparts = self.downsample[0].forward_stats(xr)
+            rbn = self.downsample[1]
+            if V.tail_deferrable(y, r, self.bn2, rbn):
+                return V.DeferredTail(y, parts, self.bn2, r, rparts, rbn)
+            return V.batchnorm_act(y, self.bn2, parts, relu=True, res=r, res_bn=rbn,
+                                   res_parts=rparts)
         return _conv_bn_act(self.conv2, self.bn2, h, res_conv=self.downsample[0],
                             res_bn=self.downsample[1], res_x=xr, twin=self.twin_out)
 
@@ -149,7 +158,22 @@
         blocks += [block(self._cin, planes, 1, dilation) for _ in range(1, count)]
         return nn.Sequential(*blocks)
 
-    def forward_features(self, x):
+    def _tail_gap_ok(self):
+        last = self.layer4[-1]
+        head = self.conv_seg
+        if not (self.training and torch.is_grad_enabled() and type(last) is BasicBlock
+                and last.downsample is not None and type(head) is Lyr.Sequential):
+            return False
+        if not V.tail_gap_on():
+            return False
+        mm = torch.nn.modules.module
+        if mm._global_forward_hooks or mm._global_forward_pre_hooks:
+            return False
+        watched = [self, last, head, *head._modules.values()]
+        return not (self.layer4._forward_hooks or
+                    any(m._forward_hooks or m._forward_pre_hooks for m in watched))
+
+    def forward_features(self, x, defer_tail=False):
         if self.conv1.weight.is_cuda and not _eval_fused_ok(self, x):
             V.prepack(self)
         V.clear_twins()
@@ -157,10 +181,18 @@
         mp = self.maxpool
         x = V.batchnorm_relu_maxpool(y, self.bn1, parts, mp.kernel_size, mp.stride, mp.padding,
                                      twin=True)
-        return self.layer4(self.layer3(self.layer2(self.layer1(x))))
+        x = self.layer3(self.layer2(self.layer1(x)))
+        if not defer_tail:
+            return self.layer4(x)
+        last = self.layer4[-1]
+        last.defer_tail = True
+        try:
+            return self.layer4(x)
+        finally:
+            last.defer_tail = False
 
     def forward(self, x):
-        return self.conv_seg(self.forward_features(x))
+        return self.conv_seg(self.forward_features(x, self._tail_gap_ok()))
 
 
 def resnet(depth, **kw):
diff --git a/multimodal_alzheimer_amd/volume_ops.py b/multimodal_alzheimer_amd/volume_ops.py
--- a/multimodal_alzheimer_amd/volume_ops.py
+++ b/multimodal_alzheimer_amd/volume_ops.py
@@ -789,16 +789,61 @@
 _BN_DUAL = os.environ.get("MMAD_BN_DUAL", "1") != "0"
 
 
+def pair_mask_on():
+    return L.load().mmad_set_kernel_variant(b"pair_mask", -1) != 0
+
+
+def tail_gap_on():
+    return L.load().mmad_set_kernel_variant(b"tail_gap", -1) != 0
+
+
+class DeferredTail:
+
+    def __init__(self, y, parts, bn, res, res_parts, res_bn):
+        self.y, self.parts, self.bn = y, parts, bn
+        self.res, self.res_parts, self.res_bn = res, res_parts, res_bn
+
+    shape = property(lambda self: self.y.shape)
+    dtype = property(lambda self: self.y.dtype)
+    device = property(lambda self: self.y.device)
+    is_cuda = property(lambda self: self.y.is_cuda)
+
+    def dim(self):
+        return self.y.dim()
+
+    def materialize(self):
+        return batchnorm_act(self.y, self.bn, self.parts, relu=True, res=self.res,
+                             res_bn=self.res_bn, res_parts=self.res_parts)
+
+
+def materialize(x):
+    return x.materialize() if isinstance(x, DeferredTail) else x
+
+
+def tail_deferrable(y, res, bn, res_bn):
+    return (y.is_cuda and tail_gap_on() and _BN_DUAL and GAP_BCAST and torch.is_grad_enabled()
+            and y.dim() == 5 and y.dtype == torch.bfloat16 and y.requires_grad
+            and res.shape == y.shape and res.dtype == y.dtype
+            and bn.training and res_bn.training
+            and _mask_from_y_ok(y) and y.numel() // y.shape[1] < 2 ** 31)
+
+
 def _bn_backward_pair(g, relu_out, y, mean, invstd, gamma, batch_stats, y2, mean2, invstd2,
-                      gamma2, batch_stats2, params, params2, g2=None, g_rows=0):
+                      gamma2, batch_stats2, params, params2, g2=None, g_rows=0, affine=None):
     m, c = _rows(y)
     dev = y.device
     dt = L.dtype_code(y.dtype)
     nparts = L.load().mmad_bn_bwd_parts(m, c)
     parts = torch.empty((2, nparts, 2, c), dtype=torch.float32, device=dev)
-    L.call("mmad_bn_bwd_reduce2", dt, m, c, L.ptr(g), L.ptr(g2), g_rows, L.ptr(relu_out),
-           L.ptr(y), L.ptr(mean), L.ptr(invstd), L.ptr(y2), L.ptr(mean2), L.ptr(invstd2),
-           L.ptr(parts[0]), L.ptr(parts[1]), L.stream())
+    if affine is not None:
+        aff = [L.ptr(t) for t in affine]
+        L.call("mmad_bn_bwd_reduce2_affine", dt, m, c, L.ptr(g), L.ptr(g2), g_rows, *aff,
+               L.ptr(y), L.ptr(mean), L.ptr(invstd), L.ptr(y2), L.ptr(mean2), L.ptr(invstd2),
+               L.ptr(parts[0]), L.ptr(parts[1]), L.stream())
+    else:
+        L.call("mmad_bn_bwd_reduce2", dt, m, c, L.ptr(g), L.ptr(g2), g_rows, L.ptr(relu_out),
+               L.ptr(y), L.ptr(mean), L.ptr(invstd), L.ptr(y2), L.ptr(mean2), L.ptr(invstd2),
+               L.ptr(parts[0]), L.ptr(parts[1]), L.stream())
     dgamma = grad_slot(params[0], (c,), dev)
     dbeta = grad_slot(params[1], (c,), dev)
     dgamma2 = grad_slot(params2[0], (c,), dev)
@@ -810,9 +855,14 @@
            L.ptr(coef[1]), L.stream())
     dy = torch.empty_like(y)
     dy2 = torch.empty_like(y2)
-    L.call("mmad_bn_bwd_apply2", dt, m, c, L.ptr(g), L.ptr(g2), g_rows, L.ptr(relu_out),
-           L.ptr(y), L.ptr(mean), L.ptr(invstd), L.ptr(coef[0]), L.ptr(dy), L.ptr(y2),
-           L.ptr(mean2), L.ptr(invstd2), L.ptr(coef[1]), L.ptr(dy2), L.stream())
+    if affine is not None:
+        L.call("mmad_bn_bwd_apply2_affine", dt, m, c, L.ptr(g), L.ptr(g2), g_rows, *aff,
+               L.ptr(y), L.ptr(mean), L.ptr(invstd), L.ptr(coef[0]), L.ptr(dy), L.ptr(y2),
+               L.ptr(mean2), L.ptr(invstd2), L.ptr(coef[1]), L.ptr(dy2), L.stream())
+    else:
+        L.call("mmad_bn_bwd_apply2", dt, m, c, L.ptr(g), L.ptr(g2), g_rows, L.ptr(relu_out),
+               L.ptr(y), L.ptr(mean), L.ptr(invstd), L.ptr(coef[0]), L.ptr(dy), L.ptr(y2),
+               L.ptr(mean2), L.ptr(invstd2), L.ptr(coef[1]), L.ptr(dy2), L.stream())
     return dy, dgamma, dbeta, dy2, dgamma2, dbeta2
 
 
@@ -839,8 +889,12 @@
         masky = relu and res is None and y.dim() == 5 and _mask_from_y_ok(y)
         if masky and bnsum and not twin and y.dtype == torch.bfloat16:
             _BNSUM_SRC[id(out)] = (weakref.ref(out), (y, mean, invstd, scale, shift))
-        ctx.save_for_backward(y, out if relu and not masky else None, mean, invstd, gamma,
-                              res if rbn is not None else None, rmean, rinvstd, rgamma)
+        pairmask = (rbn is not None and _BN_DUAL and relu and _mask_from_y_ok(y)
+                    and pair_mask_on())
+        aff = (scale, shift, rscale, rshift) if pairmask else (None,) * 4
+        ctx.save_for_backward(y, out if relu and not masky and not pairmask else None, mean,
+                              invstd, gamma, res if rbn is not None else None, rmean, rinvstd,
+                              rgamma, *aff)
         ctx.mask_affine = (scale, shift) if masky else None
         ctx.cfg = (relu, batch, rbatch, res is not None, rbn is not None)
         ctx.params = ((gamma, beta), (rgamma, rbeta))
@@ -851,10 +905,11 @@
 
     @staticmethod
     def backward(ctx, g, g2=None):
-        y, out, mean, invstd, gamma, rres, rmean, rinvstd, rgamma = ctx.saved_tensors
+        y, out, mean, invstd, gamma, rres, rmean, rinvstd, rgamma, *aff = ctx.saved_tensors
         relu, batch, rbatch, has_res, has_rbn = ctx.cfg
-        pair = (has_rbn and _BN_DUAL and out is not None and ctx.mask_affine is None
-                and _mask_from_y_ok(y))
+        affine = tuple(aff) if aff[0] is not None else None
+        pair = affine is not None or (has_rbn and _BN_DUAL and out is not None
+                                      and ctx.mask_affine is None and _mask_from_y_ok(y))
         g_rows = _gap_rows(g, y) if pair and y.numel() // y.shape[1] < 2 ** 31 else 0
         if g_rows:
             g2 = _twin_grads(g2, None, y)[0]
@@ -867,7 +922,7 @@
             rg = None if rgamma is None else rgamma.detach()
             dy, dgamma, dbeta, dres, drg, drb = _bn_backward_pair(
                 g, out, y, mean, invstd, gam, batch, rres, rmean, rinvstd, rg, rbatch,
-                ctx.params[0], ctx.params[1], g2, g_rows)
+                ctx.params[0], ctx.params[1], g2, g_rows, affine)
             return (dy, None, dgamma if ctx.needs_input_grad[2] else None,
                     dbeta if ctx.needs_input_grad[3] else None, dres, None,
                     drg if ctx.needs_input_grad[6] else None,
```

After: 2819 volumes/sec, median of 6. About the same (+0.5%).
